# inksci/TRPO

Measured on AMD Instinct MI355X. Metric: TRPO updates/sec (10-iter CG + linesearch) at N states; FVP GB/s vs HBM peak, higher is better.
Workload: dtype fp32 (f16x3 split); 1 GPU; C4: 8M states, obs 128, 256x256 tanh MLP, 18 actions; full update = discount+standardise+pg+10 CG+shs FVP+line search+final losses; n_states=8000000, obs_dim=128, n_actions=18, num_params=103442, cg_iters=10, parallelism=dp1 (row shards, RCCL all-reduce of [P] FVP/grad + loss scalars)

## Files before the change

include/trpo_engine.h:

```cpp
#ifndef TRPO_ENGINE_H
#define TRPO_ENGINE_H

#include <stdint.h>

#ifdef __cplusplus
extern "C" {
#endif

#define TRPO_MEM_HOST 0
#define TRPO_MEM_DEVICE 1

#define TRPO_OK 0
#define TRPO_ERR_ARG (-1)
#define TRPO_ERR_HIP (-2)
#define TRPO_ERR_RCCL (-3)
#define TRPO_ERR_STATE (-4)

typedef struct trpo_engine trpo_engine;

typedef struct trpo_update_params {
  int cg_iters;
  float residual_tol;
  float cg_damping;
  double max_kl;
// ... 9 lines not shown
  double shs, lm, rate;
  float surr_before, kl_before, ent_before;
  float surr_after, kl_after, ent_after;
  float rdotr;
  float gdotstepdir;
} trpo_update_stats;

#define TRPO_VEC_THETA 0
#define TRPO_VEC_THETA_PREV 1
#define TRPO_VEC_G 2
#define TRPO_VEC_STEPDIR 3
#define TRPO_VEC_FULLSTEP 4
#define TRPO_VEC_THETA_LS 5


int trpo_create(trpo_engine** out, int obs_dim, const int* hidden, int n_hidden, int n_actions,
                int64_t max_rows, int device);
void trpo_destroy(trpo_engine* e);
const char* trpo_last_error(void);
int64_t trpo_num_params(const trpo_engine* e);
int trpo_synchronize(trpo_engine* e);
void* trpo_stream(trpo_engine* e);

int trpo_comm_unique_id(uint8_t out_id[128]);
int trpo_comm_init(trpo_engine* e, const uint8_t id[128], int rank, int world);
typedef int (*trpo_allreduce_cb)(void* host_buf, int64_t count, int dtype, void* ctx);
int trpo_comm_set_host_allreduce(trpo_engine* e, trpo_allreduce_cb cb, void* ctx, int rank, int world);
typedef struct trpo_comm_info_t {
  int transport;
  int rank, world;
  int comm_count, comm_rank, comm_device;
  int device;
  char pci_bus_id[64];
} trpo_comm_info_t;
int trpo_comm_info(trpo_engine* e, trpo_comm_info_t* out);

int trpo_set_flat(trpo_engine* e, const float* theta, int mem);
int trpo_get_flat(trpo_engine* e, float* theta_out, int mem);
int trpo_get_vector(trpo_engine* e, int which, float* out, int mem);

int trpo_set_batch(trpo_engine* e, int64_t n, int64_t n_global, const float* states,
                   const int64_t* actions, const float* advant, const float* old_dist, int mem);
int trpo_set_rewards(trpo_engine* e, const double* rewards, const uint8_t* episode_starts,
                     const double* baseline, int mem);
int trpo_compute_advantages(trpo_engine* e, double gamma, double* returns_out, double* advant_out,
                            int mem);

int trpo_standardize(trpo_engine* e, double* adv, int64_t n, int64_t n_global, float* adv32_out, int mem);

#define TRPO_ADV_RETURNS 0
#define TRPO_ADV_GAE 1
int trpo_set_advantage_estimator(trpo_engine* e, int kind, double lambda);
int trpo_get_advantage_estimator(trpo_engine* e, int* kind, double* lambda);
int trpo_set_tail_values(trpo_engine* e, const double* tail_values, int mem);
int trpo_get_tail_values(trpo_engine* e, double* out, int mem);

int trpo_losses(trpo_engine* e, float out3[3]);
int trpo_eval_losses(trpo_engine* e, const float* theta, float out3[3], int mem);
int trpo_action_dist(trpo_engine* e, float* out, int mem);
int trpo_policy_grad(trpo_engine* e, float* g_out, int mem);
int trpo_fvp(trpo_engine* e, const float* v, float* out, float damping, int mem);

int trpo_cg(trpo_engine* e, const float* b, float* x_out, int cg_iters, float residual_tol,
            float damping, int* iters_out, int mem);
#define TRPO_F32 0
#define TRPO_F64 1
typedef int (*trpo_fax_cb)(const void* p, void* z, void* ctx);
int trpo_cg_callback(trpo_fax_cb f_Ax, void* ctx, const void* b, void* x_out, int64_t n, int dtype,
                     int cg_iters, double residual_tol, int* iters_out);
int trpo_linesearch(trpo_engine* e, const float* x, const float* fullstep, double expected_improve_rate,
                    float* theta_out, int* k_out, int mem);

void trpo_default_params(trpo_update_params* p);
int trpo_update(trpo_engine* e, const trpo_update_params* p, trpo_update_stats* stats);

int trpo_device_count(int* out);
int trpo_discount(const double* x, const uint8_t* episode_starts, int64_t n, double gamma,
                  double* out, int mem);
int trpo_gae(const double* rewards, const double* values, const uint8_t* episode_starts,
             const double* tail_values, int64_t n, double gamma, double lambda, double* adv_out,
             double* returns_out, int mem);

int trpo_set_option(const char* name, int value);
int trpo_get_option(const char* name, int* value);

int trpo_profile_enable(trpo_engine* e, int enable);
int trpo_profile_query(trpo_engine* e, char* buf, int cap);
int trpo_profile_reset(trpo_engine* e);

typedef struct trpo_rollout_params {
  int n_envs;
  int max_pathlength;
  int64_t n_timesteps;
  int train;
  int time_limit;
  uint64_t seed;
  const double* reset_uniforms;
  const double* action_uniforms;
  int max_episodes_per_env;
  int mem;
} trpo_rollout_params;
void trpo_default_rollout_params(trpo_rollout_params* p);
int trpo_rollout_cartpole(trpo_engine* e, const trpo_rollout_params* p, int64_t* n_steps_out, int64_t* n_paths_out);
int trpo_rollout_fetch(trpo_engine* e, double* obs, float* obs32, int64_t* actions, float* action_dists,
                       double* rewards, uint8_t* episode_starts, double* uniforms, int mem);
int trpo_rollout_fetch_ends(trpo_engine* e, uint8_t* truncated, double* final_obs, float* final_dists,
                            int64_t* lengths, int64_t* end_rows, int mem);
int trpo_rollout_to_batch(trpo_engine* e, int64_t n_global);
typedef struct trpo_feed_view {
  int64_t n, n_global;
  int obs_dim, n_actions;
  const float* states;
  int ld_states;
  const float* old_dist;
  int ld_old;
  const uint8_t* episode_starts;
  const double* returns;
  double* baseline;
} trpo_feed_view;
int trpo_get_feed_view(trpo_engine* e, trpo_feed_view* out);
typedef struct trpo_tail_view {
  int64_t n, n_paths;
  int obs_dim, n_actions;
  const float* final_obs32;
  const float* final_dist;
  const int64_t* lengths;
  const uint8_t* truncated;
  const int64_t* end_rows;
  double* tail;
} trpo_tail_view;
int trpo_get_tail_view(trpo_engine* e, trpo_tail_view* out);
int trpo_set_baseline(trpo_engine* e, const double* baseline, int mem);
int trpo_explained_variance(trpo_engine* e, double* out);
int trpo_act(trpo_engine* e, const float* states, int64_t n, const double* uniforms, int train, int64_t* actions_out,
             float* dists_out, int mem);
int trpo_cat_sample(const float* prob, int64_t n, int k, const double* uniforms, int64_t* out, int mem);
int trpo_cartpole_step(const double* state, const int64_t* action, int64_t n, double* state_out, double* reward,
                       uint8_t* done, int mem);

typedef struct trpo_vf trpo_vf;
int trpo_vf_create(trpo_vf** out, int feat_dim, const int* hidden, int n_hidden, int64_t max_rows, int device);
void trpo_vf_destroy(trpo_vf* vf);
int64_t trpo_vf_num_params(const trpo_vf* vf);
int trpo_vf_set_params(trpo_vf* vf, const float* flat, int mem);
int trpo_vf_get_params(trpo_vf* vf, float* flat_out, int mem);
int trpo_vf_set_adam(trpo_vf* vf, float lr, float beta1, float beta2, float epsilon);
int trpo_vf_reset_optimizer(trpo_vf* vf);
int trpo_vf_get_optimizer(trpo_vf* vf, float* m_out, float* v_out, float powers_out[2], int64_t* steps_out,
                          int mem);
int trpo_vf_set_features(trpo_vf* vf, int64_t n, int64_t n_global, const float* obs, int obs_dim,
                         const float* action_dists, int n_actions, const uint8_t* episode_starts, int mem);
int trpo_vf_set_features_view(trpo_vf* vf, const trpo_feed_view* view, int with_targets);
int trpo_vf_set_feature_matrix(trpo_vf* vf, int64_t n, int64_t n_global, const float* feat, int mem);
int trpo_vf_get_feature_matrix(trpo_vf* vf, float* feat_out, int mem);
int trpo_vf_set_targets(trpo_vf* vf, const void* returns, int dtype, int mem);
int trpo_vf_fit(trpo_vf* vf, int steps);
int trpo_vf_gradient(trpo_vf* vf, float* grad_out, double* loss_out, int mem);
int trpo_vf_predict(trpo_vf* vf, void* out, int dtype, int mem);
int trpo_vf_predict_tails(trpo_vf* vf, const trpo_tail_view* view);
int trpo_vf_comm_init(trpo_vf* vf, const uint8_t id[128], int rank, int world);
int trpo_vf_comm_set_host_allreduce(trpo_vf* vf, trpo_allreduce_cb cb, void* ctx, int rank, int world);

#ifdef __cplusplus
}
#endif
#endif
// ... 1 lines not shown
```

trpo_amd/_lib.py:

```python
from __future__ import annotations

import ctypes
import os
from ctypes import (CFUNCTYPE, POINTER, byref, c_char_p, c_double, c_float, c_int, c_int64, c_uint8,
                    c_void_p)

HERE = os.path.dirname(os.path.abspath(__file__))
LIB_PATH = os.environ.get("TRPO_ENGINE_LIB", os.path.join(HERE, "libtrpo_engine.so"))

MEM_HOST = 0
MEM_DEVICE = 1

VEC_THETA, VEC_THETA_PREV, VEC_G, VEC_STEPDIR, VEC_FULLSTEP, VEC_THETA_LS = range(6)

ADV_RETURNS, ADV_GAE = 0, 1


class UpdateParams(ctypes.Structure):
    _fields_ = [("cg_iters", c_int), ("residual_tol", c_float), ("cg_damping", c_float),
                ("max_kl", c_double), ("compute_advantages", c_int), ("gamma", c_double)]


class UpdateStats(ctypes.Structure):
    _fields_ = [("cg_iters", c_int), ("k", c_int), ("reverted", c_int), ("pad", c_int),
                ("shs", c_double), ("lm", c_double), ("rate", c_double),
                ("surr_before", c_float), ("kl_before", c_float), ("ent_before", c_float),
                ("surr_after", c_float), ("kl_after", c_float), ("ent_after", c_float),
                ("rdotr", c_float), ("gdotstepdir", c_float)]

    def as_dict(self):
        return {name: getattr(self, name) for name, _ in self._fields_ if name != "pad"}


class RolloutParams(ctypes.Structure):
    _fields_ = [("n_envs", c_int), ("max_pathlength", c_int), ("n_timesteps", c_int64), ("train", c_int),
                ("time_limit", c_int), ("seed", ctypes.c_uint64), ("reset_uniforms", c_void_p),
                ("action_uniforms", c_void_p), ("max_episodes_per_env", c_int), ("mem", c_int)]


class CommInfo(ctypes.Structure):
    _fields_ = [("transport", c_int), ("rank", c_int), ("world", c_int), ("comm_count", c_int),
                ("comm_rank", c_int), ("comm_device", c_int), ("device", c_int), ("pci_bus_id", ctypes.c_char * 64)]


class FeedView(ctypes.Structure):
    _fields_ = [("n", c_int64), ("n_global", c_int64), ("obs_dim", c_int), ("n_actions", c_int),
                ("states", c_void_p), ("ld_states", c_int), ("old_dist", c_void_p), ("ld_old", c_int),
                ("episode_starts", c_void_p), ("returns", c_void_p), ("baseline", c_void_p)]


class TailView(ctypes.Structure):
    _fields_ = [("n", c_int64), ("n_paths", c_int64), ("obs_dim", c_int), ("n_actions", c_int),
                ("final_obs32", c_void_p), ("final_dist", c_void_p), ("lengths", c_void_p),
                ("truncated", c_void_p), ("end_rows", c_void_p), ("tail", c_void_p)]


FAX_CB = CFUNCTYPE(c_int, c_void_p, c_void_p, c_void_p)
ALLREDUCE_CB = CFUNCTYPE(c_int, c_void_p, c_int64, c_int, c_void_p)
F32, F64 = 0, 1

SIGNATURES = {
    "trpo_create": (c_int, [POINTER(c_void_p), c_int, POINTER(c_int), c_int, c_int, c_int64, c_int]),
    "trpo_destroy": (None, [c_void_p]),
    "trpo_last_error": (c_char_p, []),
    "trpo_num_params": (c_int64, [c_void_p]),
    "trpo_synchronize": (c_int, [c_void_p]),
    "trpo_stream": (c_void_p, [c_void_p]),
    "trpo_comm_unique_id": (c_int, [POINTER(c_uint8)]),
    "trpo_comm_init": (c_int, [c_void_p, POINTER(c_uint8), c_int, c_int]),
    "trpo_comm_set_host_allreduce": (c_int, [c_void_p, ALLREDUCE_CB, c_void_p, c_int, c_int]),
    "trpo_comm_info": (c_int, [c_void_p, ctypes.POINTER(CommInfo)]),
    "trpo_set_flat": (c_int, [c_void_p, c_void_p, c_int]),
    "trpo_get_flat": (c_int, [c_void_p, c_void_p, c_int]),
    "trpo_get_vector": (c_int, [c_void_p, c_int, c_void_p, c_int]),
    "trpo_set_batch": (c_int, [c_void_p, c_int64, c_int64, c_void_p, c_void_p, c_void_p, c_void_p, c_int]),
    "trpo_set_rewards": (c_int, [c_void_p, c_void_p, c_void_p, c_void_p, c_int]),
    "trpo_compute_advantages": (c_int, [c_void_p, c_double, c_void_p, c_void_p, c_int]),
    "trpo_standardize": (c_int, [c_void_p, c_void_p, c_int64, c_int64, c_void_p, c_int]),
    "trpo_set_advantage_estimator": (c_int, [c_void_p, c_int, c_double]),
    "trpo_get_advantage_estimator": (c_int, [c_void_p, POINTER(c_int), POINTER(c_double)]),
    "trpo_set_tail_values": (c_int, [c_void_p, c_void_p, c_int]),
    "trpo_get_tail_values": (c_int, [c_void_p, c_void_p, c_int]),
    "trpo_losses": (c_int, [c_void_p, POINTER(c_float)]),
    "trpo_eval_losses": (c_int, [c_void_p, c_void_p, POINTER(c_float), c_int]),
    "trpo_action_dist": (c_int, [c_void_p, c_void_p, c_int]),
    "trpo_policy_grad": (c_int, [c_void_p, c_void_p, c_int]),
    "trpo_fvp": (c_int, [c_void_p, c_void_p, c_void_p, c_float, c_int]),
    "trpo_cg": (c_int, [c_void_p, c_void_p, c_void_p, c_int, c_float, c_float, POINTER(c_int), c_int]),
    "trpo_cg_callback": (c_int, [FAX_CB, c_void_p, c_void_p, c_void_p, c_int64, c_int, c_int, c_double,
                                 POINTER(c_int)]),
    "trpo_linesearch": (c_int, [c_void_p, c_void_p, c_void_p, c_double, c_void_p, POINTER(c_int), c_int]),
    "trpo_default_params": (None, [POINTER(UpdateParams)]),
    "trpo_update": (c_int, [c_void_p, POINTER(UpdateParams), POINTER(UpdateStats)]),
    "trpo_device_count": (c_int, [POINTER(c_int)]),
    "trpo_discount": (c_int, [c_void_p, c_void_p, c_int64, c_double, c_void_p, c_int]),
    "trpo_gae": (c_int, [c_void_p, c_void_p, c_void_p, c_void_p, c_int64, c_double, c_double, c_void_p, c_void_p,
                         c_int]),
    "trpo_set_option": (c_int, [c_char_p, c_int]),
    "trpo_get_option": (c_int, [c_char_p, POINTER(c_int)]),
    "trpo_profile_enable": (c_int, [c_void_p, c_int]),
    "trpo_profile_query": (c_int, [c_void_p, c_char_p, c_int]),
    "trpo_profile_reset": (c_int, [c_void_p]),
    "trpo_default_rollout_params": (None, [POINTER(RolloutParams)]),
    "trpo_rollout_cartpole": (c_int, [c_void_p, POINTER(RolloutParams), POINTER(c_int64), POINTER(c_int64)]),
    "trpo_rollout_fetch": (c_int, [c_void_p, c_void_p, c_void_p, c_void_p, c_void_p, c_void_p, c_void_p, c_void_p,
                                   c_int]),
    "trpo_rollout_fetch_ends": (c_int, [c_void_p, c_void_p, c_void_p, c_void_p, c_void_p, c_void_p, c_int]),
    "trpo_get_tail_view": (c_int, [c_void_p, POINTER(TailView)]),
    "trpo_vf_predict_tails": (c_int, [c_void_p, POINTER(TailView)]),
    "trpo_set_baseline": (c_int, [c_void_p, c_void_p, c_int]),
    "trpo_get_feed_view": (c_int, [c_void_p, POINTER(FeedView)]),
    "trpo_vf_set_features_view": (c_int, [c_void_p, POINTER(FeedView), c_int]),
    "trpo_explained_variance": (c_int, [c_void_p, POINTER(c_double)]),
    "trpo_rollout_to_batch": (c_int, [c_void_p, c_int64]),
    "trpo_act": (c_int, [c_void_p, c_void_p, c_int64, c_void_p, c_int, c_void_p, c_void_p, c_int]),
    "trpo_cat_sample": (c_int, [c_void_p, c_int64, c_int, c_void_p, c_void_p, c_int]),
    "trpo_cartpole_step": (c_int, [c_void_p, c_void_p, c_int64, c_void_p, c_void_p, c_void_p, c_int]),
    "trpo_vf_create": (c_int, [POINTER(c_void_p), c_int, POINTER(c_int), c_int, c_int64, c_int]),
    "trpo_vf_destroy": (None, [c_void_p]),
    "trpo_vf_num_params": (c_int64, [c_void_p]),
    "trpo_vf_set_params": (c_int, [c_void_p, c_void_p, c_int]),
    "trpo_vf_get_params": (c_int, [c_void_p, c_void_p, c_int]),
    "trpo_vf_set_adam": (c_int, [c_void_p, c_float, c_float, c_float, c_float]),
    "trpo_vf_reset_optimizer": (c_int, [c_void_p]),
    "trpo_vf_get_optimizer": (c_int, [c_void_p, c_void_p, c_void_p, POINTER(c_float), POINTER(c_int64), c_int]),
    "trpo_vf_set_features": (c_int, [c_void_p, c_int64, c_int64, c_void_p, c_int, c_void_p, c_int, c_void_p,
                                     c_int]),
    "trpo_vf_set_feature_matrix": (c_int, [c_void_p, c_int64, c_int64, c_void_p, c_int]),
    "trpo_vf_get_feature_matrix": (c_int, [c_void_p, c_void_p, c_int]),
    "trpo_vf_set_targets": (c_int, [c_void_p, c_void_p, c_int, c_int]),
    "trpo_vf_fit": (c_int, [c_void_p, c_int]),
    "trpo_vf_gradient": (c_int, [c_void_p, c_void_p, POINTER(c_double), c_int]),
    "trpo_vf_predict": (c_int, [c_void_p, c_void_p, c_int, c_int]),
    "trpo_vf_comm_init": (c_int, [c_void_p, POINTER(c_uint8), c_int, c_int]),
    "trpo_vf_comm_set_host_allreduce": (c_int, [c_void_p, ALLREDUCE_CB, c_void_p, c_int, c_int]),
}


class EngineError(RuntimeError):
    pass


def _load():
    if not os.path.isfile(LIB_PATH):
        raise ImportError(
            f"trpo_amd: HIP engine library not found at {LIB_PATH}; build it with "
            f"`python -c 'import __graft_entry__ as g; g.build()'` (there is no CPU fallback)")
    try:
        lib = ctypes.CDLL(LIB_PATH)
    except OSError as exc:
        raise ImportError(f"trpo_amd: failed to load {LIB_PATH}: {exc}") from exc
    for name, (res, args) in SIGNATURES.items():
        fn = getattr(lib, name)
        fn.restype = res
        fn.argtypes = args
    return lib


lib = _load()


def check(rc: int, what: str = ""):
    if rc != 0:
        msg = lib.trpo_last_error()
        raise EngineError(f"{what} failed (rc={rc}): {msg.decode() if msg else ''}")
    return rc


def device_count() -> int:
    n = c_int(0)
    check(lib.trpo_device_count(ctypes.byref(n)), "trpo_device_count")
    return n.value


def set_option(name: str, value: int):
    check(lib.trpo_set_option(name.encode(), int(value)), f"trpo_set_option({name})")


def get_option(name: str) -> int:
    out = c_int(0)
    check(lib.trpo_get_option(name.encode(), byref(out)), f"trpo_get_option({name})")
# ... 2 lines not shown
```

trpo_amd/csrc/engine.cpp:

```cpp
#include "../../include/trpo_engine.h"
#include "abi_util.h"
#include "common.h"
#include "kernels.h"

#include <hip/hip_runtime.h>
#include <rccl/rccl.h>

#include <algorithm>
#include <cmath>
#include <cstddef>
#include <cstdio>
#include <cstdlib>
#include <cstring>
#include <map>
#include <memory>
#include <stdexcept>
#include <string>
#include <type_traits>
#include <vector>

using namespace trpo;

using namespace trpo_abi;

// ... 81 lines not shown
    void rd_written() { ds_ready = false; }
  } cache;

  bool f16 = false;
  unsigned* amax = nullptr;
  unsigned* am(int group, int l) const {
    return f16 ? amax + (size_t)(1 + group * kMaxLayers + l) * kAmaxSlot : nullptr;
  }
  unsigned* am_x() const { return f16 ? amax : nullptr; }
  unsigned* am_w(int l) const { return am(0, l); }
  unsigned* am_v(int l) const { return am(1, l); }
  unsigned* am_d(int l) const { return am(3, l); }
  unsigned* am_ds(int l) const { return am(4, l); }
  unsigned* am_rh(int l) const { return am(5, l); }
  unsigned* am_rd(int l) const { return am(6, l); }
  void am_reset(unsigned* first, int count) {
    if (first && count > 0)
      HIPCHECK(hipMemsetAsync(first, 0, (size_t)count * kAmaxSlot * sizeof(unsigned), stream));
  }
  uint16_t *Xh = nullptr, *Xl = nullptr, *W0b = nullptr, *V0b = nullptr;
  int* pl_e = nullptr;
  uint16_t* D1h = nullptr;
  int d1_ldp = 0;
  int* eD1t = nullptr;
  bool use_hbwd2() const {
    return g_options.hbwd2 != 0 && L >= 3 && wp[L - 1] > 128 && head_bwd2_eligible(w[L], wp[L - 1]);
  }
  int x_mpad = 0, x_ldp = 0;
  bool x_planes = false;
  bool planes_geom_l0() const {
    return L >= 2 && wp[1] % 256 == 0 && r16(wp[0]) % 64 == 0;
  }
  bool f16_split() const { return f16 && split_on(); }
  bool x_planes_on() const { return x_planes && g_options.planes != 0 && split_on(); }
  bool planes_l0() const { return x_planes_on() && planes_geom_l0() && rowgemm_uses_split(wp[1], RowEpi::kTanh); }
  bool rbwd0_geom() const { return L >= 2 && rbwd0_eligible(wp[0], (wp[0] + 63) / 64 * 64, wp[1], wp[2]); }
  void attach_x_planes(GemmSeg& sg, uint16_t* dst) {
    launch_block_planes(sg.B3, 2, wp[1], r16(wp[0]), dst, stream);
    sg.Ah = Xh;
    sg.Al = Xl;
    sg.ldp = x_ldp;
    sg.mpad = x_mpad;
    sg.eAp = pl_e;
    sg.Bb = dst;
  }
  uint16_t* tail_planes = nullptr;
  bool use_tail() const {
    return g_options.tail != 0 && f16_split() && L >= 2 && tail_eligible(wp[L - 1], wp[L]) && w[L] <= 32;
  }
  bool e_top_needed() const { return L < 2 || !use_tail() || use_fused() || use_chain(); }
  void reprepare_if_path_changed() {
    if (cache.prepared && ((e_top_needed() && !cache.prep_e_top) || cache.prep_fused16 != use_fused16()))
      cache.prepared = false;
  }

  struct ImageSet {
    uint16_t* img = nullptr;
    int* tab = nullptr;
    int* e = nullptr;
    int nchunks = 0;
    ChainImgArgs jobs{};
  };
  int chain_otm = 0;
  ImageSet chain_set;
  bool use_fused() const { return g_options.fused != 0 && chain_otm > 0 && fused_fvp_eligible(L, w.data()); }
  ImageSet f16_set;
  bool f16_v_img_ready = false;
  unsigned* cg_ticket = nullptr;
  ImageSet f16_loss_set;
  bool use_fused16() const { return g_options.fused == 3 && f16 && f16_set.img && fused16_eligible(L, w.data()); }
  uint16_t* rf_img = nullptr;
  uint16_t* fw_img = nullptr;
  bool use_rfwd01() const {
    return g_options.rfwd01 != 0 && rf_img && f16_split() && use_tail() && planes_l0() &&
           rfwd01_eligible(L, w.data(), wp.data()) && rfwd01_rows_ok(x_mpad);
  }
  bool use_fwd01() const {
    return g_options.fwd01 != 0 && fw_img && f16_split() && planes_l0() && fwd01_eligible(L, w.data(), wp.data()) &&
           rfwd01_rows_ok(x_mpad);
  }
  bool use_rbwd0() const {
    return g_options.rbwd0 != 0 && f16 && x_planes_on() && rbwd0_geom() && rowgemm_uses_split(wp[1], RowEpi::kRBwd);
  }
  RBwd0Args rbwd0_args(const int* skip) const {
    RBwd0Args a{};
    a.rows = (int)n;
    a.K = wp[2];
    a.lda = wp[2];
    a.N = w[1];
    a.Npad = wp[1];
    a.obs = w[0];
    a.B0 = WB3[1];
    a.B1 = WB3[1] + 3 * plane3_b(1);
    a.ldk = r16(wp[2]);
    a.plane = (int64_t)plane3_b(1);
    a.am_b0 = am_w(1);
    a.am_b1 = am_v(1);
    a.H = H[1];
    a.Xh = Xh;
    a.Xl = Xl;
    a.x_mpad = x_mpad;
    a.x_ldp = x_ldp;
    a.eX = pl_e;
    a.dst = slab_dst(0);
    a.skip = skip;
    return a;
  }
  bool use_chain() const {
    return chain_otm > 0 && (g_options.chain >= 2 || (g_options.chain == 1 && chain_otm <= 8));
  }

  struct RollBufs {
    std::vector<void*> mem;
    int64_t rows = 0;
    int envs = 0;
    double* obs = nullptr;
    int64_t* actions = nullptr;
    float* dist = nullptr;
    double* rewards = nullptr;
    uint8_t* starts = nullptr;
    double* uniforms = nullptr;
    int64_t *counts = nullptr, *episodes = nullptr, *offsets = nullptr;
    double *reset_u = nullptr, *act_u = nullptr;
    int64_t reset_u_n = 0, act_u_n = 0;
    int64_t paths = 0;
    uint8_t* end_truncated = nullptr;
    double* end_obs = nullptr;
    float* end_dist = nullptr;
    int64_t *end_len = nullptr, *end_row = nullptr, *path_offsets = nullptr;
    uint8_t* cat_truncated = nullptr;
    float *cat_obs32 = nullptr, *cat_dist = nullptr;
    int64_t *cat_len = nullptr, *cat_rows = nullptr;
  } roll;
  RolloutArgs roll_args{};
  int64_t roll_n = 0, roll_paths = 0, roll_maxcount = 0, roll_maxpaths = 0;
  bool roll_valid = false;
  bool feed_is_rollout = false;

  bool prof = false;
  struct Ev {
    std::string tag;
    hipEvent_t a, b;
  };
  std::vector<Ev> ev_live;
  std::vector<hipEvent_t> ev_pool;
  std::map<std::string, std::pair<long, double>> prof_acc;

  template <class T>
  T* dalloc(size_t count) {
    void* ptr = nullptr;
    const size_t bytes = std::max<size_t>(count * sizeof(T), 16);
    HIPCHECK(hipMalloc(&ptr, bytes));
    HIPCHECK(hipMemsetAsync(ptr, 0, bytes, stream));
    allocs.push_back(ptr);
    return static_cast<T*>(ptr);
  }

  void use() {
    HIPCHECK(hipSetDevice(device));
    if (!har_slots.empty()) rewind_har();
  }

  const float* act_in(int l) const { return l == 0 ? X : H[l]; }

  hipEvent_t take_event() {
    if (!ev_pool.empty()) {
// ... 18 lines not shown
      if (e->prof) begin(std::string(prefix) + "_l" + std::to_string(l));
    }
    void begin(const std::string& tag) {
      Ev ev{tag, e->take_event(), e->take_event()};
      HIPCHECK(hipEventRecord(ev.a, e->stream));
      e->ev_live.push_back(ev);
      idx = (int)e->ev_live.size() - 1;
    }
    ~Scope() {
      if (idx >= 0) (void)hipEventRecord(e->ev_live[idx].b, e->stream);
    }
  };
  void prof_collect() {
    if (ev_live.empty()) return;
    HIPCHECK(hipStreamSynchronize(stream));
    for (auto& ev : ev_live) {
      float ms = 0.f;
      HIPCHECK(hipEventElapsedTime(&ms, ev.a, ev.b));
      auto& acc = prof_acc[ev.tag];
      acc.first += 1;
      acc.second += ms;
      ev_pool.push_back(ev.a);
      ev_pool.push_back(ev.b);
    }
    ev_live.clear();
  }

  void init(int obs, const int* hidden, int nh, int A, int64_t max_rows, int dev) {
    REQUIRE(obs > 0 && A > 0 && nh >= 0 && max_rows > 0, "invalid policy dimensions");
    REQUIRE(nh + 1 <= kMaxLayers, "too many layers");
    REQUIRE(A <= 32 * kMaxHeadTiles, "n_actions must be <= 128 (softmax rows of up to 4 x 32 lanes)");
    REQUIRE(max_rows < (int64_t(1) << 31), "max_rows must fit in int32 row indices");
    for (int i = 0; i < nh; ++i) REQUIRE(hidden[i] > 0, "hidden widths must be positive");
    device = dev;
    use();
    HIPCHECK(hipDeviceGetAttribute(&num_cus, hipDeviceAttributeMultiprocessorCount, device));
    HIPCHECK(hipStreamCreateWithFlags(&stream, hipStreamNonBlocking));
    w.push_back(obs);
    for (int i = 0; i < nh; ++i) w.push_back(hidden[i]);
    w.push_back(A);
    L = (int)w.size() - 1;
    for (int v : w) wp.push_back(pad4(v));
    P = 0;
    for (int l = 0; l < L; ++l) {
      offW.push_back(P);
      P += (int64_t)w[l] * w[l + 1];
      offb.push_back(P);
      P += w[l + 1];
    }
    cap = max_rows;

    for (float** v : {&theta, &theta_prev, &theta_trial, &theta_ls, &g, &bneg, &x, &r, &p, &p2, &z, &hv,
                      &stepdir, &fullstep, &vin, &vout})
      *v = dalloc<float>(P);
    int maxpad = 4;
    for (int l = 0; l < L; ++l) {
      WF.push_back(dalloc<float>((size_t)2 * wp[l] * wp[l + 1]));
      WB.push_back(dalloc<float>((size_t)2 * wp[l + 1] * wp[l]));
      WFt.push_back(dalloc<float>((size_t)2 * wp[l] * wp[l + 1]));
      maxpad = std::max<int>(maxpad, 2 * wp[l] * wp[l + 1]);
    }
    WBt_scratch = dalloc<float>(maxpad);
    for (int l = 0; l < L; ++l) {
      WF3.push_back(dalloc<uint16_t>(2 * plane3_f(l) * 3));
      WB3.push_back(dalloc<uint16_t>(2 * plane3_b(l) * 3));
      WFt3.push_back(dalloc<uint16_t>(plane3_f(l) * 3));
    }
    X = dalloc<float>((size_t)cap * wp[0]);
    act = dalloc<int>(cap);
    adv32 = dalloc<float>(cap);
    old = dalloc<float>((size_t)cap * wp[L]);
    rewards = dalloc<double>(cap);
    returns = dalloc<double>(cap);
    adv64 = dalloc<double>(cap);
    baseline = dalloc<double>(cap);
    starts = dalloc<uint8_t>(cap);
    H.assign(L + 1, nullptr);
    RH.assign(L + 1, nullptr);
    D.assign(L, nullptr);
    RD.assign(L, nullptr);
    E.assign(L, nullptr);
    for (int l = 1; l < L; ++l) {
      H[l] = dalloc<float>((size_t)cap * wp[l]);
      RH[l] = dalloc<float>((size_t)cap * wp[l]);
    }
    for (int l = 0; l < L; ++l) {
      D[l] = dalloc<float>((size_t)cap * wp[l + 1]);
      RD[l] = dalloc<float>((size_t)cap * wp[l + 1]);
      if (l < L - 1) E[l] = dalloc<float>((size_t)cap * wp[l + 1]);
    }
    Pm = dalloc<float>((size_t)cap * wp[L]);
    DSL = dalloc<float>((size_t)cap * wp[L]);
    rowterms = dalloc<double>((size_t)cap * 4);
    int tiles_max = 1;
    for (int l = 0; l < L; ++l)
      tiles_max = std::max(tiles_max, ((w[l] + 255) / 256) * ((w[l + 1] + 255) / 256));
    slab_stride = (P + 63) / 64 * 64;
    int s_target = std::max(1, std::min(512, 1024 / tiles_max));
    if (tiles_max == 1)
      s_target = (int)std::max<int64_t>(s_target, std::min<int64_t>(2048, (int64_t(128) << 20) / (slab_stride * 4)));
    const int64_t slab_bytes = (int64_t)slab_stride * 4;
    auto fit = [&](int64_t bytes) { return std::max<int64_t>(1, bytes / slab_bytes); };
    s_target = (int)std::max<int64_t>(s_target, std::min<int64_t>(fit(int64_t(2) << 30), (cap + 16383) / 16384));
    if (tiles_max == 1 && s_target == 512 && num_cus < 512 && (cap + 16383) / 16384 <= num_cus) s_target = num_cus;
    if (g_options.splits > 0) s_target = std::min(g_options.splits, 8192);
    int s_pg = (int)std::max<int64_t>(
        s_target, std::min<int64_t>({2048, std::max<int64_t>(4 * (int64_t)s_target, (cap + 4095) / 4096),
                                     fit(int64_t(8) << 30)}));
    if (g_options.pg_splits > 0) s_pg = std::min(g_options.pg_splits, 8192);
    slab = dalloc<float>((size_t)std::max(s_target, s_pg) * slab_stride);
    S = s_target;
    S_pg = s_pg;
    S_cur = S;
    partA = dalloc<double>(kRedBlocks * 3);
    partB = dalloc<double>(kRedBlocks * 3);
    part3 = dalloc<double>(kRedBlocks * 3);
    local3 = dalloc<double>(4);
    dscal = dalloc<double>(8);
    scan_ws = dalloc<uint8_t>(std::max(discount_workspace_bytes(cap), gae_workspace_bytes(cap)));
    sc = dalloc<UpdScalars>(1);
    fl = dalloc<CGFlags>(1);
    cg_ticket = dalloc<unsigned>(1);
    dbad = dalloc<int>(1);
    f16 = g_options.split_f16 != 0;
    amax = dalloc<unsigned>((size_t)(1 + 8 * kMaxLayers) * kAmaxSlot);
    if (L >= 2 && tail_eligible(wp[L - 1], wp[L])) tail_planes = dalloc<uint16_t>((size_t)2 * 2 * 32 * kTailK);
    if (rfwd01_eligible(L, w.data(), wp.data())) rf_img = dalloc<uint16_t>(rfwd01_img_bytes() / 2);
    if (fwd01_eligible(L, w.data(), wp.data())) fw_img = dalloc<uint16_t>(fwd01_img_bytes() / 2);
    stage = dalloc<float>((size_t)cap * std::max(std::max(wp[0], wp[L]), 2));
    if (f16 && (planes_geom_l0() || rbwd0_geom())) {
      x_ldp = (wp[0] + 63) / 64 * 64;
      const size_t xp = (size_t)((cap + 255) / 256 * 256) * x_ldp;
      Xh = dalloc<uint16_t>(xp);
      Xl = dalloc<uint16_t>(xp);
      W0b = dalloc<uint16_t>(2 * plane3_f(0));
      V0b = dalloc<uint16_t>(2 * plane3_f(0));
      pl_e = dalloc<int>(8);
    }
    if (f16 && L >= 2 && rbwd0_geom()) {
      d1_ldp = (wp[2] + 31) / 32 * 32;
      D1h = dalloc<uint16_t>((size_t)((cap + 255) / 256 * 256) * d1_ldp);
      eD1t = dalloc<int>((size_t)(cap + 31) / 32 + 8);
    }
    HIPCHECK(hipHostMalloc((void**)&hsc, sizeof(UpdScalars), hipHostMallocDefault));
    std::memset(hsc, 0, sizeof(UpdScalars));
    setup_chain();
    setup_fused16();
    HIPCHECK(hipStreamSynchronize(stream));
  }

  struct ImgJob {
    int l, trans, which;
  };
  struct ImgGeom {
    int kc, otp, csz;
  };
  std::vector<ImgJob> fvp_image_order() const {
    std::vector<ImgJob> order = {ImgJob{0, 0, 1}};
    for (int l = 1; l < L; ++l) {
      order.push_back({l, 0, 0});
      order.push_back({l, 0, 1});
    }
    for (int l = L - 1; l >= 1; --l) {
      order.push_back({l, 1, 0});
      order.push_back({l, 1, 1});
    }
    return order;
// ... 555 lines not shown
      if (l == L - 1 && hb2) {
        am_reset(am_ds(L - 2), 1);
        HeadBwd2Args hb{};
        hb.rows = (int)n;
        hb.A = w[L];
        hb.Apad = wp[L];
        hb.N = w[L - 1];
        hb.Npad = wp[L - 1];
        hb.WB = WB[L - 1];
        hb.D2 = D[L - 1];
        hb.DS2 = DSL;
        hb.H = H[L - 1];
        hb.D1 = D[L - 2];
        hb.DS1 = RD[L - 2];
        hb.E1 = prep_e_top ? E[L - 2] : nullptr;
        hb.am_d1 = am_d(L - 2);
        hb.am_ds1 = am_ds(L - 2);
        PgSplits pgs(this);
        hb.dst = slab_dst(L - 1);
        if (L == 3 && D1h && eD1t && use_rbwd0() && wp[2] % 32 == 0 && n > 0) {
          cache.d1_mpad = (int)((n + 255) / 256 * 256);
          hb.D1h = D1h;
          hb.d1_mpad = cache.d1_mpad;
          hb.eD1t = eD1t;
        }
        Scope sp(this, "bwd2_l2");
        launch_head_bwd2(hb, num_cus, stream);
        check_launch();
        cache.ds_ready = true;
        cache.d1_plane = cache.d1_tiled = hb.D1h != nullptr;
        continue;
      }
      RowGemmArgs a = row_args(w[l], wp[l]);
      a.nseg = 1;
      a.seg[0] = bwd_seg(l, kW, D[l], am_d(l));
      a.epi = need_d ? (need_e ? RowEpi::kPrepBwd : RowEpi::kPgBwd) : RowEpi::kPrepBwdE;
      a.ea.H = H[l];
      a.ea.out0 = need_d ? D[l - 1] : E[l - 1];
      a.ea.amax0 = need_d ? am_d(l - 1) : nullptr;
      a.ea.out1 = need_d && need_e ? E[l - 1] : nullptr;
      a.ea.ldo = wp[l];
      Scope sp(this, "bwd", l);
      launch_rowgemm(a, stream);
      check_launch();
    }
    if (!cache.d1_plane && D1h && use_rbwd0() && n > 0) {
      cache.d1_mpad = (int)((n + 255) / 256 * 256);
      Scope sp(this, "split_d1");
      launch_split_planes(D[1], (int)n, cache.d1_mpad, wp[2], wp[2], D1h, nullptr, d1_ldp, am_d(1), pl_e + 1, stream);
      check_launch();
      cache.d1_plane = true;
    }
    reduce_losses(0, nullptr);
    cache.prepared = true;
  }

  void reduce_grad(float* out, const int* skip, int slabs = 0) {
    {
      Scope sp(this, "reduce");
      launch_reduce_slab(slab, slabs > 0 ? slabs : active_splits, slab_stride, P, out, skip, stream);
      check_launch();
    }
    allreduce_f32(out, (size_t)P);
  }

  void wgrad_layer(int l, int nseg, WSeg s0, WSeg s1, int colsum_seg, const int* skip, const char* tag) {
    WGradArgs a{};
    a.rows = (int)n;
    a.Ma = w[l];
    a.Nb = w[l + 1];
    a.Mpad = wp[l];
    a.Npad = wp[l + 1];
    a.nseg = nseg;
    a.seg[0] = s0;
    a.seg[1] = s1;
    a.colsum_seg = colsum_seg;
    a.dst = slab_dst(l);
    a.skip = skip;
    a.f16 = f16;
    Scope sp(this, tag, l);
    launch_wgrad(a, stream);
    check_launch();
  }
  void fvp_wgrads(int l0, int l1, const int* skip) {
    for (int l = l0; l < l1; ++l) {
      if (l == 0)
        wgrad_layer(0, 1, WSeg{X, RD[0], wp[0], wp[1], am_x(), am_rd(0)}, WSeg{}, 0, skip, "fvp_wgrad");
      else
        wgrad_layer(l, 2, WSeg{RH[l], D[l], wp[l], wp[l + 1], am_rh(l), am_d(l)},
                    WSeg{H[l], RD[l], wp[l], wp[l + 1], nullptr, am_rd(l)}, 1, skip, "fvp_wgrad");
    }
  }

  void policy_grad() {
    reprepare_if_path_changed();
    prepare();
    if (use_fused16()) {
      if (!cache.pg_ready) pg_fused16();
      reduce_grad(g, nullptr, cache.pg_grid);
      return;
    }
    ensure_w3();
    PgSplits pgs(this);
    cache.slabs_written(true);
    std::vector<float*> DS(L);
    DS[L - 1] = DSL;
    for (int l = 0; l < L - 1; ++l) DS[l] = RD[l];
    const bool have_ds = cache.ds_ready;
    am_reset(am_ds(0), have_ds ? L - 2 : L - 1);
    const bool r0f = use_rbwd0();
    for (int l = have_ds ? L - 2 : L - 1; l >= 1; --l) {
      if (l == 1 && r0f) {
        RBwd0Args a = rbwd0_args(nullptr);
        a.nseg = 1;
        a.A0 = DS[1];
        a.am_a0 = am_ds(1);
        Scope sp(this, "pg_bwdwg_l1");
        launch_rbwd0(a, stream);
        check_launch();
        continue;
      }
      RowGemmArgs a = row_args(w[l], wp[l]);
      a.nseg = 1;
      a.seg[0] = bwd_seg(l, kW, DS[l], am_ds(l));
      a.epi = RowEpi::kPgBwd;
      a.ea.H = H[l];
      a.ea.out0 = DS[l - 1];
      a.ea.amax0 = am_ds(l - 1);
      a.ea.ldo = wp[l];
      Scope sp(this, "pg_bwd", l);
      launch_rowgemm(a, stream);
      check_launch();
    }
    for (int l = r0f ? 1 : 0; l < (have_ds ? L - 1 : L); ++l)
      wgrad_layer(l, 1, WSeg{act_in(l), DS[l], wp[l], wp[l + 1], l == 0 ? am_x() : nullptr, am_ds(l)}, WSeg{}, 0,
                  nullptr, "pg_wgrad");
    reduce_grad(g, nullptr);
  }

  void fvp(const float* v, float* out, const int* skip, int* defer = nullptr) {
    if (defer) *defer = 0;
    reprepare_if_path_changed();
    prepare();
    cache.rd_written();
    cache.slabs_written();
    if (use_fused16()) {
      fvp_fused16(v, out, skip, defer && !multi_rank() && cg_fused_reduce_ok(P) ? defer : nullptr);
      return;
    }
    if (use_fused()) {
      fvp_fused(v, out, skip);
      return;
    }
    if (use_chain()) {
      fvp_chain(v, out, skip);
      return;
    }
    {
      PackArgs pa = pack_args(WF, &WB, 1);
      launch_pack(pa, v, 1, skip, stream);
      check_launch();
    }
    ensure_w3();
    split_parts(false, true, false, true, cur_set(), skip, "split_v");
    am_reset(am_rh(0), L);
    am_reset(am_rd(0), L);
    const bool tail = use_tail();
    const int Lf = tail ? L - 1 : L;
    int l_first = 0;
    if (use_rfwd01()) {
      {
        Scope sp(this, "fvp_rfwd_img");
        launch_rfwd01_img(theta, v, offW[0], offW[1], w[0], am_v(0), am_w(1), am_v(1), rf_img, skip, stream);
        check_launch();
      }
      Rfwd01Args ra{};
      ra.n = n;
      ra.obs = w[0];
      ra.ldh = wp[1];
      ra.ldz = wp[2];
      ra.Xh = Xh;
      ra.Xl = Xl;
      ra.x_mpad = x_mpad;
      ra.eX = pl_e;
      ra.H1 = H[1];
      ra.c0 = v + offb[0];
      ra.c1 = v + offb[1];
      ra.V0 = v + offW[0];
      ra.RH1 = RH[1];
      ra.RZ2 = RH[2];
      ra.img = rf_img;
      ra.am_v0 = am_v(0);
      ra.am_w1 = am_w(1);
      ra.am_v1 = am_v(1);
      ra.am_rh1 = am_rh(1);
      ra.am_rz2 = am_rh(2);
      ra.skip = skip;
      Scope sp(this, "fvp_rfwd01");
      launch_rfwd01(ra, num_cus, stream);
      check_launch();
      l_first = 2;
    }
    for (int l = l_first; l < Lf; ++l) {
      RowGemmArgs a = row_args(w[l + 1], wp[l + 1]);
      if (l == 0) {
        a.nseg = 1;
        a.seg[0] = fwd_seg(0, kV, X, am_x(), cur_set());
        if (planes_l0()) attach_x_planes(a.seg[0], V0b);
      } else {
        a.nseg = 2;
        a.seg[0] = fwd_seg(l, kW, RH[l], am_rh(l), cur_set());
        a.seg[1] = fwd_seg(l, kV, H[l], nullptr, cur_set());
      }
      a.skip = skip;
      a.ea.bias = v + offb[l];
      a.ea.ldo = wp[l + 1];
      if (l < L - 1) {
        a.epi = (tail && l == L - 2) ? RowEpi::kRZ : RowEpi::kRHidden;
        a.ea.H = H[l + 1];
        a.ea.out0 = RH[l + 1];
        a.ea.amax0 = am_rh(l + 1);
      } else {
        a.epi = RowEpi::kRHead;
        a.ea.P = Pm;
        a.ea.out0 = RD[L - 1];
        a.ea.amax0 = am_rd(L - 1);
        a.ea.invN = 1.0 / (double)n_global;
      }
      Scope sp(this, "fvp_rfwd", l);
      launch_rowgemm(a, stream);
      check_launch();
    }
    if (tail) {
      const int l = L - 1;
      TailPackArgs tp{};
      tp.theta = theta;
      tp.v = v;
      tp.off_w = offW[l];
      tp.a = w[l];
      tp.b = w[l + 1];
      tp.am_w = am_w(l);
      tp.am_v = am_v(l);
      tp.out = tail_planes;
      TailArgs ta{};
      ta.rows = (int)n;
      ta.a = w[l];
      ta.b = w[l + 1];
      ta.apad = wp[l];
      ta.bpad = wp[l + 1];
      ta.RH = RH[l];
      ta.rz = 1;
      ta.H = H[l];
      ta.P = Pm;
      ta.DL = D[l];
      ta.c = v + offb[l];
      ta.WV16 = tail_planes;
      ta.WT16 = WB3[l];
      ta.VT16 = WB3[l] + 3 * plane3_b(l);
      ta.bplane = (int64_t)plane3_b(l);
      ta.am_rh = am_rh(l);
      ta.am_d = am_d(l);
      ta.am_w = am_w(l);
      ta.am_v = am_v(l);
      ta.am_out = am_rd(l - 1);
      ta.RDout = RD[l - 1];
      ta.invN = 1.0 / (double)n_global;
      ta.dst = slab_dst(l);
      ta.skip = skip;
      Scope sp(this, "fvp_tail", l);
      launch_tail_pack(tp, stream);
      launch_fvp_tail(ta, stream);
      check_launch();
    }
    const bool r0f = use_rbwd0() && Lf - 1 >= 1;
    for (int l = Lf - 1; l >= 1; --l) {
      if (l == 1 && r0f) {
        RBwd0Args a = rbwd0_args(skip);
        a.nseg = 2;
        a.A0 = RD[1];
        a.A1 = D[1];
        if (cache.d1_plane) {
          a.A1h = D1h;
          a.a1_mpad = cache.d1_mpad;
          a.eA1p = pl_e + 1;
          if (cache.d1_tiled) a.eA1t = eD1t;
        }
        a.am_a0 = am_rd(1);
        a.am_a1 = am_d(1);
        a.E = E[0];
        a.RH = RH[1];
        Scope sp(this, "fvp_rbwdwg_l1");
        launch_rbwd0(a, stream);
        check_launch();
        continue;
      }
      RowGemmArgs a = row_args(w[l], wp[l]);
      a.nseg = 2;
      a.seg[0] = bwd_seg(l, kW, RD[l], am_rd(l));
      a.seg[1] = bwd_seg(l, kV, D[l], am_d(l));
      a.skip = skip;
      a.epi = RowEpi::kRBwd;
      a.ea.H = H[l];
      a.ea.E = E[l - 1];
      a.ea.RH = RH[l];
      a.ea.out0 = RD[l - 1];
      a.ea.amax0 = am_rd(l - 1);
      a.ea.ldo = wp[l];
      Scope sp(this, "fvp_rbwd", l);
      launch_rowgemm(a, stream);
      check_launch();
    }
    fvp_wgrads(r0f ? 1 : 0, Lf, skip);
    reduce_grad(out, skip);
  }

  ChainArgs chain_args(const ImageSet& is, const float* v, const int* skip) const {
    ChainArgs ca{};
    ca.n = (int)n;
    ca.L = L;
    for (int l = 0; l <= L; ++l) {
      ca.w[l] = w[l];
      ca.ld[l] = wp[l];
    }
    ca.X = X;
    for (int l = 0; l < L; ++l) {
      ca.H[l] = H[l];
      ca.RH[l] = RH[l];
      ca.D[l] = D[l];
      ca.E[l] = E[l];
      ca.RD[l] = RD[l];
      ca.offb[l] = offb[l];
    }
    ca.P = Pm;
    ca.v = v;
    ca.img = is.img;
    ca.tab = is.tab;
    ca.nchunks = is.nchunks;
    ca.invN = 1.0 / (double)n_global;
    ca.skip = skip;
    return ca;
  }
  void chain_w_images(const float* v) {
    if (cache.chain_w_valid) return;
    Scope sp(this, "fvp_img_w");
    launch_chain_img(chain_set.jobs, theta, v, 0, nullptr, stream);
    check_launch();
    cache.chain_w_valid = true;
  }
  void chain_images(const float* v, const int* skip) {
    chain_w_images(v);
    Scope sp(this, "fvp_img_v");
    launch_chain_img(chain_set.jobs, theta, v, 1, skip, stream);
    check_launch();
  }

  void fvp_fused(const float* v, float* out, const int* skip) {
    chain_images(v, skip);
    const int variant = g_options.fused == 1 ? 1 : 2;
    const int rb = fused_fvp_states_per_group(variant);
    FusedArgs fa{};
    fa.c = chain_args(chain_set, v, skip);
    fa.slab = slab;
    fa.slab_stride = slab_stride;
    for (int l = 0; l < L; ++l) fa.offW[l] = offW[l];
    fa.ngroups = (int)((n + rb - 1) / rb);
    const int per_cu = variant == 2 ? 2 : 1;
    const int grid =
        (int)std::max<int64_t>(1, std::min<int64_t>({(int64_t)fa.ngroups, (int64_t)S, (int64_t)num_cus * per_cu}));
    {
      Scope sp(this, "fvp_fused");
      launch_fvp_fused(fa, grid, variant, stream);
      check_launch();
    }
    reduce_grad(out, skip, grid);
  }

  Fused16Args fused16_args(const float* v, const int* skip, int& grid) {
    const int rb = fused16_states_per_group();
    Fused16Args fa{};
    fa.f.c = chain_args(f16_set, v, skip);
    fa.f.slab = slab;
    fa.f.slab_stride = slab_stride;
    for (int l = 0; l < L; ++l) fa.f.offW[l] = offW[l];
    fa.f.ngroups = (int)((n + rb - 1) / rb);
    fa.img_e = f16_set.e;
    fa.am_x = am_x();
    fa.am_d1 = am_d(1);
    fa.am_d2 = L == 3 ? am_d(2) : nullptr;
    fa.DS = DSL;
    fa.am_ds2 = am_ds(L - 1);
    const int64_t slots = std::max<int64_t>(
        1, std::min<int64_t>({(int64_t)fa.f.ngroups, (int64_t)S, (int64_t)num_cus * fused16_groups_per_cu()}));
    const int64_t rounds = (fa.f.ngroups + slots - 1) / slots;
    grid = (int)std::max<int64_t>(1, (fa.f.ngroups + rounds - 1) / rounds);
    return fa;
// ... 1083 lines not shown
```

trpo_amd/csrc/gemm.hip:

```cpp
#include "common.h"
#include "kernels.h"
#include <cstdlib>
#include <stdexcept>
#include <type_traits>
#include <string>

#include "rowepi.h"

namespace trpo {

static int env_int(const char* name, int dflt) {
  const char* e = std::getenv(name);
  return e ? std::atoi(e) : dflt;
}
Options g_options = {env_int("TRPO_SPLIT_MFMA", 5), env_int("TRPO_SPLIT_WG", 1), env_int("TRPO_CHAIN", 1),
                     env_int("TRPO_SPLIT_F16", 1), env_int("TRPO_SPLIT_MIN_K", 0), env_int("TRPO_GRAPHS", 1),
                     env_int("TRPO_TAIL", 1), env_int("TRPO_FUSED", 3), env_int("TRPO_LOW_SEG", 14),
                     env_int("TRPO_PLANES", 1), env_int("TRPO_RBWD0", 1), env_int("TRPO_HBWD2", 2),
                     env_int("TRPO_HEAD_FWD", 1), env_int("TRPO_SPLITS", 0),
                     env_int("TRPO_PG_SPLITS", 0), env_int("TRPO_LS_FUSED", 1),
                     env_int("TRPO_CG_FUSE_REDUCE", 1), env_int("TRPO_CG_P_IMG", 1),
                     env_int("TRPO_RFWD01", 1), env_int("TRPO_FWD01", 1)};

namespace {

template <int WM, int WN, int TM, int TN, int BK, int EPI, int PF = 1>
__global__ void __launch_bounds__(WM* WN * 64, (TM * TN >= 8 || EPI == 2) ? 2 : 4)
rowgemm_kernel(const RowGemmArgs args) {
  constexpr int BM = WM * TM * 32, BN = WN * TN * 32, NT = WM * WN * 64;
  constexpr int LDA = BK + 4;
  constexpr int LDB = BN + 4;
  constexpr int ASZ = BM * LDA, BSZ = BK * LDB;
  __shared__ __attribute__((aligned(16))) float smem[2 * (ASZ + BSZ)];
  if (args.skip && *args.skip) return;

  const int tid = threadIdx.x, lane = tid & 63, wave = tid >> 6;
  const int wm = wave % WM, wn = wave / WM;
  const int lr = lane & 31, lh = lane >> 5;
  int mt, ntile;
  tile_of((args.Npad + BN - 1) / BN, mt, ntile);
  const int m0 = mt * BM, n0 = ntile * BN;
  const int M = args.M;

  const int nt0 = (args.seg[0].K + BK - 1) / BK;
  const int nt1 = args.nseg > 1 ? (args.seg[1].K + BK - 1) / BK : 0;
  const int ntiles = nt0 + nt1;

  f32x16 acc[TM][TN];
#pragma unroll
  for (int i = 0; i < TM; ++i)
#pragma unroll
    for (int j = 0; j < TN; ++j) acc[i][j] = f32x16{};

  constexpr int AF4 = BM * BK / 4, BF4 = BK * BN / 4;
  constexpr int AP = (AF4 + NT - 1) / NT, BP = (BF4 + NT - 1) / NT;
  struct Stage {
    f32x4 ra[AP], rb[BP];
    bool oka[AP], okb[BP];
  };

  auto gload = [&](Stage& st, int t) {
    const bool s1 = t >= nt0;
    const float* Ap = s1 ? args.seg[1].A : args.seg[0].A;
    const float* Bp = s1 ? args.seg[1].B : args.seg[0].B;
    const int lda = s1 ? args.seg[1].lda : args.seg[0].lda;
    const int ldb = s1 ? args.seg[1].ldb : args.seg[0].ldb;
    const int K = s1 ? args.seg[1].K : args.seg[0].K;
    const int k0 = (s1 ? t - nt0 : t) * BK;
#pragma unroll
    for (int i = 0; i < AP; ++i) {
      const int f = tid + i * NT;
      const int r = f / (BK / 4), kq = f % (BK / 4);
      const int row = m0 + r, k = k0 + 4 * kq;
      const bool ok = (AF4 % NT == 0 || f < AF4) && row < M && k < K;
      st.ra[i] = *reinterpret_cast<const f32x4*>(Ap + (size_t)(ok ? row : 0) * lda + (ok ? k : 0));
      st.oka[i] = ok;
    }
#pragma unroll
    for (int i = 0; i < BP; ++i) {
      const int f = tid + i * NT;
      const int kr = f / (BN / 4), cq = f % (BN / 4);
      const int k = k0 + kr, col = n0 + 4 * cq;
      const bool ok = (BF4 % NT == 0 || f < BF4) && k < K && col < args.Npad;
      st.rb[i] = *reinterpret_cast<const f32x4*>(Bp + (size_t)(ok ? k : 0) * ldb + (ok ? col : 0));
      st.okb[i] = ok;
    }
  };
  auto sstore = [&](const Stage& st, int buf) {
    float* As = smem + buf * (ASZ + BSZ);
    float* Bs = As + ASZ;
#pragma unroll
    for (int i = 0; i < AP; ++i) {
      const int f = tid + i * NT;
      if (AF4 % NT == 0 || f < AF4) {
        const int r = f / (BK / 4), kq = f % (BK / 4);
        *reinterpret_cast<f32x4*>(As + r * LDA + 4 * kq) = st.oka[i] ? st.ra[i] : f32x4{};
      }
    }
#pragma unroll
    for (int i = 0; i < BP; ++i) {
      const int f = tid + i * NT;
      if (BF4 % NT == 0 || f < BF4) {
        const int kr = f / (BN / 4), cq = f % (BN / 4);
        *reinterpret_cast<f32x4*>(Bs + kr * LDB + 4 * cq) = st.okb[i] ? st.rb[i] : f32x4{};
      }
// ... 240 lines not shown
          c = __builtin_amdgcn_mfma_f32_32x32x16_bf16(a[1], b[1], c, 0, 0, 0);
          c = __builtin_amdgcn_mfma_f32_32x32x16_bf16(a[2], b[0], c, 0, 0, 0);
          c = __builtin_amdgcn_mfma_f32_32x32x16_bf16(a[0], b[2], c, 0, 0, 0);
          c = __builtin_amdgcn_mfma_f32_32x32x16_bf16(a[1], b[0], c, 0, 0, 0);
          c = __builtin_amdgcn_mfma_f32_32x32x16_bf16(a[0], b[1], c, 0, 0, 0);
          c = __builtin_amdgcn_mfma_f32_32x32x16_bf16(a[0], b[0], c, 0, 0, 0);
          acc[tm][tn] = c;
        }
      } else {
        f16x8 b[2];
#pragma unroll
        for (int p = 0; p < 2; ++p) b[p] = *reinterpret_cast<const f16x8*>(Bs + p * BPL + bo);
#pragma unroll
        for (int tm = 0; tm < TM; ++tm) {
          f16x8 a[2];
          const int ao = swk(wm * TM * 32 + tm * 32 + lr, 2 * ks + lh);
#pragma unroll
          for (int p = 0; p < 2; ++p) a[p] = *reinterpret_cast<const f16x8*>(As + p * APL + ao);
          f32x16 c = acc[tm][tn];
          c = __builtin_amdgcn_mfma_f32_32x32x16_f16(a[1], b[0], c, 0, 0, 0);
          c = __builtin_amdgcn_mfma_f32_32x32x16_f16(a[0], b[1], c, 0, 0, 0);
          c = __builtin_amdgcn_mfma_f32_32x32x16_f16(a[0], b[0], c, 0, 0, 0);
          acc[tm][tn] = c;
        }
      }
    }
  };
  auto compute = [&](int buf, int t) {
    if (t >= nt0 ? one1 : one0) compute_p(buf, std::true_type{});
    else compute_p(buf, std::false_type{});
  };
  auto seg_switch = [&](int t) {
    if constexpr (NP == 2) {
      if (t == nt0 && nt1 > 0) {
        asm volatile("; segment switch" ::: "memory");
        scale_acc<TM, TN>(acc, eP1 - eP0);
      }
    }
  };

  if (ntiles > 0) {
    if constexpr (PF == 1) {
      Stage S;
      gload(S, 0);
      sstore(S, 0);
      lds_barrier();
      for (int t = 0; t < ntiles; ++t) {
        if (t + 1 < ntiles) gload(S, t + 1);
        seg_switch(t);
        compute(t & 1, t);
        if (t + 1 < ntiles) sstore(S, (t + 1) & 1);
        lds_barrier();
      }
    } else {
      Stage S0, S1;
      gload(S0, 0);
      gload(S1, ntiles > 1 ? 1 : 0);
      sstore(S0, 0);
      lds_barrier();
      int t = 0;
      for (; t + 1 < ntiles; t += 2) {
        gload(S0, t + 2 < ntiles ? t + 2 : ntiles - 1);
        seg_switch(t);
        compute(0, t);
        sstore(S1, 1);
        lds_barrier();
        gload(S1, t + 3 < ntiles ? t + 3 : ntiles - 1);
        seg_switch(t + 1);
        compute(1, t + 1);
        if (t + 2 < ntiles) sstore(S0, 0);
        lds_barrier();
      }
      if (t < ntiles) {
        seg_switch(t);
        compute(0, t);
      }
    }
  }
  if constexpr (NP == 2) scale_acc<TM, TN>(acc, -(nt1 > 0 ? eP1 : eP0));
  row_epilogue<WM, WN, TM, TN, EPI>(args, acc, m0, n0, wm, wn, lr, lh);
}


template <int WM, int WN, int TM, int TN, int OCC, int PF, int NP>
__global__ void __launch_bounds__(WM* WN * 64, OCC)
wgrad3_kernel(const WGradArgs args) {
  constexpr int BK = 16;
  constexpr int BM = WM * TM * 32, BN = WN * TN * 32, NT = WM * WN * 64;
  constexpr int APL = BM * BK, BPL = BN * BK;
  constexpr int STG = NP * (APL + BPL);
  __shared__ __attribute__((aligned(16))) unsigned short smem[2 * STG];
  __shared__ float cs_sh[2][BN];
  if (args.skip && *args.skip) return;

  const int tid = threadIdx.x, lane = tid & 63, wave = tid >> 6;
  const int wm = wave % WM, wn = wave / WM;
  const int lr = lane & 31, lh = lane >> 5;
  const int m0 = blockIdx.x * BM, n0 = blockIdx.y * BN, split = blockIdx.z;
  const int r0 = split * args.dst.rows_per_split;
  const int r1 = min(args.rows, r0 + args.dst.rows_per_split);
  const int nk = r1 > r0 ? (r1 - r0 + BK - 1) / BK : 0;
  const int ntiles = nk * args.nseg;
  const bool do_colsum = (blockIdx.x == 0);
  int eA[2] = {0, 0}, eB[2] = {0, 0};
  if constexpr (NP == 2) {
    for (int g = 0; g < args.nseg && g < 2; ++g) {
      eA[g] = amax_exp(args.seg[g].amaxA);
      eB[g] = amax_exp(args.seg[g].amaxB);
    }
  }
  bool one0 = false, one1 = false;
  if constexpr (NP == 2) {
    if (args.low_seg > 0 && args.nseg > 1) {
      const int d = (eA[1] + eB[1]) - (eA[0] + eB[0]);
      const int pen0 = (!args.seg[0].amaxA || !args.seg[0].amaxB) ? 4 : 0;
      const int pen1 = (!args.seg[1].amaxA || !args.seg[1].amaxB) ? 4 : 0;
      one0 = -d >= args.low_seg + pen1;
      one1 = d >= args.low_seg + pen0;
    }
  }

  f32x16 acc[TM][TN];
#pragma unroll
  for (int i = 0; i < TM; ++i)
#pragma unroll
    for (int j = 0; j < TN; ++j) acc[i][j] = f32x16{};

  constexpr int AI = 2 * BM, BI = 2 * BN;
  constexpr int AP = (AI + NT - 1) / NT, BP = (BI + NT - 1) / NT;
  float csum[BP];
#pragma unroll
  for (int i = 0; i < BP; ++i) csum[i] = 0.0f;
  auto desc = [&](const float* p, int ld) {
    return __builtin_amdgcn_make_buffer_rsrc((void*)(p + (size_t)r0 * ld), 0, (r1 - r0) * ld * 4, 0x00020000);
  };
  const int lda4 = args.seg[0].lda * 4, ldb4 = args.seg[0].ldb * 4;
  constexpr int kOob = 0x40000000;
  int vA[AP], vB[BP];
#pragma unroll
  for (int i = 0; i < AP; ++i) {
    const int f = tid + i * NT;
    const int c = f % BM, g = f / BM;
    const bool okc = (AI % NT == 0 || f < AI) && m0 + c < args.Mpad;
    vA[i] = okc ? 8 * g * lda4 + (m0 + c) * 4 : kOob;
  }
#pragma unroll
  for (int i = 0; i < BP; ++i) {
    const int f = tid + i * NT;
    const int c = f % BN, g = f / BN;
    const bool okc = (BI % NT == 0 || f < BI) && n0 + c < args.Npad;
    vB[i] = okc ? 8 * g * ldb4 + (n0 + c) * 4 : kOob;
  }
  auto ldbuf = [](__amdgpu_buffer_rsrc_t r, int vo, int so) {
    return __builtin_bit_cast(float, __builtin_amdgcn_raw_buffer_load_b32(r, vo, so, 0));
  };
  struct Stage {
    float va[AP][8], vb[BP][8];
    bool cs;
    int sg;
  };
  auto gload = [&](Stage& st, int t) {
    const int sg = t / nk;
    const int kt = t - sg * nk;
    st.cs = do_colsum && sg == args.colsum_seg;
    st.sg = sg;
    const __amdgpu_buffer_rsrc_t ra = desc(sg ? args.seg[1].A : args.seg[0].A, args.seg[0].lda);
    const __amdgpu_buffer_rsrc_t rb = desc(sg ? args.seg[1].B : args.seg[0].B, args.seg[0].ldb);
    const int sa = kt * BK * lda4, sb = kt * BK * ldb4;
    __builtin_amdgcn_sched_barrier(0);
#pragma unroll
    for (int i = 0; i < AP; ++i)
#pragma unroll
      for (int q = 0; q < 8; ++q) st.va[i][q] = ldbuf(ra, vA[i], sa + q * lda4);
#pragma unroll
    for (int i = 0; i < BP; ++i)
#pragma unroll
      for (int q = 0; q < 8; ++q) st.vb[i][q] = ldbuf(rb, vB[i], sb + q * ldb4);
    __builtin_amdgcn_sched_barrier(0);
  };
  auto put = [&](unsigned short* base, int plane_elems, int c, int g, const float (&v)[8], int e) {
    unsigned short* dst = base + swz16(c, g);
    if constexpr (NP == 2) {
      const float sc = __builtin_ldexpf(1.0f, e);
      u16x8 h, l;
#pragma unroll
      for (int q = 0; q < 8; ++q) {
        unsigned short hh, ll;
        split2h(v[q] * sc, hh, ll);
        h[q] = hh;
        l[q] = ll;
      }
      *reinterpret_cast<u16x8*>(dst) = h;
      *reinterpret_cast<u16x8*>(dst + plane_elems) = l;
    } else {
      u16x8 h, m, l;
#pragma unroll
      for (int q = 0; q < 8; ++q) {
        unsigned short hh, mm, ll;
        split3(v[q], hh, mm, ll);
        h[q] = hh;
        m[q] = mm;
        l[q] = ll;
      }
      *reinterpret_cast<u16x8*>(dst) = h;
      *reinterpret_cast<u16x8*>(dst + plane_elems) = m;
      *reinterpret_cast<u16x8*>(dst + 2 * plane_elems) = l;
    }
  };
  auto sstore = [&](const Stage& st, int buf) {
    unsigned short* As = smem + buf * STG;
    unsigned short* Bs = As + NP * APL;
#pragma unroll
    for (int i = 0; i < AP; ++i) {
      const int f = tid + i * NT;
      if (AI % NT == 0 || f < AI) put(As, APL, f % BM, f / BM, st.va[i], eA[st.sg]);
    }
#pragma unroll
    for (int i = 0; i < BP; ++i) {
      const int f = tid + i * NT;
      if (BI % NT == 0 || f < BI) {
        put(Bs, BPL, f % BN, f / BN, st.vb[i], eB[st.sg]);
        if (st.cs) {
          float cs = 0.0f;
#pragma unroll
          for (int q = 0; q < 8; ++q) cs += st.vb[i][q];
          csum[i] += cs;
        }
      }
    }
  };
  auto compute_p = [&](int buf, auto one_c) {
    constexpr bool ONE = decltype(one_c)::value;
    const unsigned short* As = smem + buf * STG;
    const unsigned short* Bs = As + NP * APL;
#pragma unroll
    for (int tn = 0; tn < TN; ++tn) {
      const int bo = swz16(wn * TN * 32 + tn * 32 + lr, lh);
      if constexpr (NP == 2 && ONE) {
        const f16x8 b0 = *reinterpret_cast<const f16x8*>(Bs + bo);
#pragma unroll
        for (int tm = 0; tm < TM; ++tm) {
          const int ao = swz16(wm * TM * 32 + tm * 32 + lr, lh);
          const f16x8 a0 = *reinterpret_cast<const f16x8*>(As + ao);
          acc[tm][tn] = __builtin_amdgcn_mfma_f32_32x32x16_f16(a0, b0, acc[tm][tn], 0, 0, 0);
        }
      } else if constexpr (NP == 3) {
        bf16x8 b[3];
#pragma unroll
        for (int p = 0; p < 3; ++p) b[p] = *reinterpret_cast<const bf16x8*>(Bs + p * BPL + bo);
#pragma unroll
        for (int tm = 0; tm < TM; ++tm) {
          bf16x8 a[3];
          const int ao = swz16(wm * TM * 32 + tm * 32 + lr, lh);
#pragma unroll
          for (int p = 0; p < 3; ++p) a[p] = *reinterpret_cast<const bf16x8*>(As + p * APL + ao);
          f32x16 c = acc[tm][tn];
          c = __builtin_amdgcn_mfma_f32_32x32x16_bf16(a[1], b[1], c, 0, 0, 0);
          c = __builtin_amdgcn_mfma_f32_32x32x16_bf16(a[2], b[0], c, 0, 0, 0);
          c = __builtin_amdgcn_mfma_f32_32x32x16_bf16(a[0], b[2], c, 0, 0, 0);
          c = __builtin_amdgcn_mfma_f32_32x32x16_bf16(a[1], b[0], c, 0, 0, 0);
          c = __builtin_amdgcn_mfma_f32_32x32x16_bf16(a[0], b[1], c, 0, 0, 0);
          c = __builtin_amdgcn_mfma_f32_32x32x16_bf16(a[0], b[0], c, 0, 0, 0);
          acc[tm][tn] = c;
        }
      } else {
        f16x8 b[2];
#pragma unroll
        for (int p = 0; p < 2; ++p) b[p] = *reinterpret_cast<const f16x8*>(Bs + p * BPL + bo);
#pragma unroll
        for (int tm = 0; tm < TM; ++tm) {
          f16x8 a[2];
          const int ao = swz16(wm * TM * 32 + tm * 32 + lr, lh);
#pragma unroll
          for (int p = 0; p < 2; ++p) a[p] = *reinterpret_cast<const f16x8*>(As + p * APL + ao);
          f32x16 c = acc[tm][tn];
          c = __builtin_amdgcn_mfma_f32_32x32x16_f16(a[1], b[0], c, 0, 0, 0);
          c = __builtin_amdgcn_mfma_f32_32x32x16_f16(a[0], b[1], c, 0, 0, 0);
          c = __builtin_amdgcn_mfma_f32_32x32x16_f16(a[0], b[0], c, 0, 0, 0);
          acc[tm][tn] = c;
        }
      }
    }
  };
  auto compute = [&](int buf, int t) {
    if (t >= nk ? one1 : one0) compute_p(buf, std::true_type{});
    else compute_p(buf, std::false_type{});
  };
  auto seg_switch = [&](int t) {
    if constexpr (NP == 2) {
      if (t == nk && args.nseg > 1) {
        asm volatile("; segment switch" ::: "memory");
        scale_acc<TM, TN>(acc, (eA[1] + eB[1]) - (eA[0] + eB[0]));
      }
    }
  };

  if (ntiles > 0) {
    if constexpr (PF == 1) {
// ... 265 lines not shown
    }
  if (do_colsum && tid < BN && n0 + tid < args.Nb) out[args.dst.off_b + n0 + tid] = csum;
}

template <int WM, int WN, int TM, int TN, int BKT, int EPI, int PF = 1>
void launch_row_cfg(const RowGemmArgs& a, hipStream_t s) {
  constexpr int BM = WM * TM * 32, BN = WN * TN * 32;
  const long nblk = (long)((a.M + BM - 1) / BM) * ((a.Npad + BN - 1) / BN);
  hipLaunchKernelGGL((rowgemm_kernel<WM, WN, TM, TN, BKT, EPI, PF>), dim3((unsigned)nblk), dim3(WM * WN * 64),
                     0, s, a);
}

template <int WM, int WN, int TM, int TN, int EPI, int OCC = 2, int PF = 1, int BKT = 16>
void launch_row3_cfg(const RowGemmArgs& a, hipStream_t s) {
  constexpr int BM = WM * TM * 32, BN = WN * TN * 32;
  for (int i = 0; i < a.nseg; ++i)
    if (!a.seg[i].B3 || a.seg[i].ldk < ((a.seg[i].K + 15) / 16) * 16 || a.seg[i].ldk % 8)
      throw std::runtime_error("split-bf16 row GEMM: segment without B planes");
  if (a.nseg > 1 && (a.seg[1].lda != a.seg[0].lda || a.seg[1].ldk != a.seg[0].ldk || a.seg[1].plane != a.seg[0].plane))
    throw std::runtime_error("split-bf16 row GEMM: segments with different strides");
  if ((int64_t)BM * a.seg[0].lda * 4 >= (int64_t(1) << 30) || (int64_t)(a.f16 ? 2 : 3) * a.seg[0].plane * 2 >= (int64_t(1) << 30))
    throw std::runtime_error("split-bf16 row GEMM: operand beyond the buffer-descriptor range");
  const long nblk = (long)((a.M + BM - 1) / BM) * ((a.Npad + BN - 1) / BN);
  RowGemmArgs b = a;
  b.low_seg = g_options.low_seg;
  if constexpr (BKT == 32) {
    for (int i = 0; i < a.nseg; ++i)
      if (a.seg[i].ldk % 32) throw std::runtime_error("split row GEMM (BK 32): B planes' ldk not a multiple of 32");
  }
  if (a.f16)
    hipLaunchKernelGGL((rowgemm3_kernel<WM, WN, TM, TN, EPI, OCC, PF, 2, BKT>), dim3((unsigned)nblk),
                       dim3(WM * WN * 64), 0, s, b);
  else if constexpr (BKT == 16)
    hipLaunchKernelGGL((rowgemm3_kernel<WM, WN, TM, TN, EPI, OCC, PF, 3, BKT>), dim3((unsigned)nblk),
                       dim3(WM * WN * 64), 0, s, a);
  else
    throw std::runtime_error("split row GEMM (BK 32): f16 planes only");
}

bool small_k_row(const RowGemmArgs& a) {
  if (g_options.split_min_k <= 0) return false;
  for (int i = 0; i < a.nseg; ++i)
    if (a.seg[i].K >= g_options.split_min_k) return false;
  return true;
}

template <int EPI>
void launch_row_epi(const RowGemmArgs& a, hipStream_t s) {
  if constexpr (epi_is_head(EPI)) {
    if (a.N > 32 * kMaxHeadTiles) throw std::runtime_error("softmax head supports at most 128 actions");
    if (a.N > 64) launch_row_cfg<4, 1, 2, 4, 16, EPI>(a, s);
    else if (a.N > 32) launch_row_cfg<4, 1, 2, 2, 16, EPI>(a, s);
    else launch_row_cfg<4, 1, 2, 1, 16, EPI>(a, s);
  } else if (rowgemm_uses_split(a.Npad, a.epi) && !small_k_row(a)) {
    bool bk32 = a.f16 != 0 && g_options.split_mfma == 5;
    for (int i = 0; i < a.nseg; ++i) bk32 = bk32 && a.seg[i].ldk % 32 == 0;
    if (bk32) launch_row3_cfg<4, 2, 2, 4, EPI, 2, 1, 32>(a, s);
    else if (g_options.split_mfma == 5 || g_options.split_mfma == 6) launch_row3_cfg<4, 2, 2, 4, EPI, 2, 2>(a, s);
    else launch_row3_cfg<2, 4, 2, 2, EPI>(a, s);
  } else {
    if (a.Npad <= 32) launch_row_cfg<4, 1, 2, 1, 16, EPI>(a, s);
    else if (a.Npad <= 64) launch_row_cfg<4, 1, 2, 2, 16, EPI>(a, s);
    else if (a.Npad <= 128) launch_row_cfg<2, 2, 2, 2, 16, EPI>(a, s);
    else launch_row_cfg<2, 4, 2, 2, 16, EPI>(a, s);
  }
}

template <int WM, int WN, int TM, int TN, int BKT = 16, int PF = 1>
void launch_wg_cfg(const WGradArgs& a, hipStream_t s) {
  constexpr int BM = WM * TM * 32, BN = WN * TN * 32;
  dim3 grid((a.Ma + BM - 1) / BM, (a.Nb + BN - 1) / BN, a.dst.splits);
  hipLaunchKernelGGL((wgrad_kernel<WM, WN, TM, TN, BKT, PF>), grid, dim3(WM * WN * 64), 0, s, a);
}

template <int WM, int WN, int TM, int TN, int OCC, int PF>
void launch_wg3_cfg(const WGradArgs& a, hipStream_t s) {
  constexpr int BM = WM * TM * 32, BN = WN * TN * 32;
  if (a.dst.rows_per_split % 16) throw std::runtime_error("split-bf16 wgrad: rows_per_split % 16");
  if (a.nseg > 1 && (a.seg[1].lda != a.seg[0].lda || a.seg[1].ldb != a.seg[0].ldb))
    throw std::runtime_error("split-bf16 wgrad: segments with different leading dimensions");
  if ((int64_t)a.dst.rows_per_split * (a.seg[0].lda > a.seg[0].ldb ? a.seg[0].lda : a.seg[0].ldb) * 4 >= (int64_t(1) << 30))
    throw std::runtime_error("split-bf16 wgrad: a split's rows exceed the 1 GiB buffer-descriptor range");
  dim3 grid((a.Ma + BM - 1) / BM, (a.Nb + BN - 1) / BN, a.dst.splits);
  WGradArgs b = a;
  b.low_seg = g_options.low_seg;
  if (a.f16)
    hipLaunchKernelGGL((wgrad3_kernel<WM, WN, TM, TN, OCC, PF, 2>), grid, dim3(WM * WN * 64), 0, s, b);
  else
    hipLaunchKernelGGL((wgrad3_kernel<WM, WN, TM, TN, OCC, PF, 3>), grid, dim3(WM * WN * 64), 0, s, a);
}

}

bool rowgemm_uses_split(int Npad, RowEpi epi) {
  return g_options.split_mfma != 0 && Npad > 128 && !epi_is_head((int)epi);
}

void launch_split_b(const SplitArgs& a, const int* skip, hipStream_t s) {
  if (a.n <= 0) return;
  int maxb = 1;
  for (int i = 0; i < a.n; ++i) {
    const SplitJob& j = a.job[i];
    if (j.ldk % 8 || j.ldk < ((j.K + 15) / 16) * 16) throw std::runtime_error("split_b: bad ldk");
    const int b = (j.Npad * (j.ldk / 8) + 255) / 256;
    maxb = b > maxb ? b : maxb;
  }
  hipLaunchKernelGGL(split_b_kernel, dim3(maxb, a.n), dim3(256), 0, s, a, skip);
}

void launch_rowgemm(const RowGemmArgs& a, hipStream_t s) {
  if (a.M <= 0) return;
  if (a.seg[0].Ah && g_options.planes != 0 && a.f16 && rowgemm_uses_split(a.Npad, a.epi) && !small_k_row(a) &&
      a.Npad % 256 == 0) {
    launch_rowgemm_planes(a, s);
    return;
  }
  switch (a.epi) {
    case RowEpi::kTanh: launch_row_epi<(int)RowEpi::kTanh>(a, s); break;
    case RowEpi::kRHidden: launch_row_epi<(int)RowEpi::kRHidden>(a, s); break;
    case RowEpi::kRZ: launch_row_epi<(int)RowEpi::kRZ>(a, s); break;
    case RowEpi::kPrepBwd: launch_row_epi<(int)RowEpi::kPrepBwd>(a, s); break;
    case RowEpi::kPgBwd: launch_row_epi<(int)RowEpi::kPgBwd>(a, s); break;
    case RowEpi::kPrepBwdE: launch_row_epi<(int)RowEpi::kPrepBwdE>(a, s); break;
    case RowEpi::kRBwd: launch_row_epi<(int)RowEpi::kRBwd>(a, s); break;
    case RowEpi::kPrepHead: launch_row_epi<(int)RowEpi::kPrepHead>(a, s); break;
    case RowEpi::kLossHead: launch_row_epi<(int)RowEpi::kLossHead>(a, s); break;
    case RowEpi::kRHead: launch_row_epi<(int)RowEpi::kRHead>(a, s); break;
    case RowEpi::kRelu: launch_row_epi<(int)RowEpi::kRelu>(a, s); break;
    case RowEpi::kReluBwd: launch_row_epi<(int)RowEpi::kReluBwd>(a, s); break;
  }
}

void launch_wgrad(const WGradArgs& a, hipStream_t s) {
  if (a.dst.splits <= 0) return;
  const int Mp = a.Ma, Np = a.Nb;
  if (Np <= 32) {
    if (Mp <= 64) launch_wg_cfg<2, 1, 1, 1>(a, s);
    else if (Mp <= 128) launch_wg_cfg<4, 1, 1, 1>(a, s);
    else launch_wg_cfg<4, 1, 2, 1>(a, s);
  } else if (Np <= 64) {
    if (Mp <= 64) launch_wg_cfg<2, 2, 1, 1>(a, s);
    else if (Mp <= 128) launch_wg_cfg<2, 1, 2, 2>(a, s);
    else launch_wg_cfg<4, 1, 2, 2>(a, s);
  } else if (Np <= 128) {
    if (Mp <= 64) launch_wg_cfg<1, 2, 2, 2>(a, s);
    else launch_wg_cfg<2, 2, 2, 2>(a, s);
  } else if (g_options.split_wg != 0) {
    if (Mp <= 128) launch_wg3_cfg<2, 4, 2, 2, 2, 1>(a, s);
    else launch_wg3_cfg<4, 2, 2, 4, 2, 1>(a, s);
  } else {
    if (Mp <= 128) launch_wg_cfg<2, 4, 2, 2>(a, s);
    else launch_wg_cfg<2, 4, 4, 2>(a, s);
  }
}

}
```

trpo_amd/csrc/kernels.h:

```cpp
#pragma once
#include <hip/hip_runtime.h>
#include <cstdint>

namespace trpo {

struct Options {
  int split_mfma;
  int split_wg;
  int chain;
  int split_f16;
  int split_min_k;
  int graphs;
  int tail;
  int fused;
  int low_seg;
  int planes;
  int rbwd0;
  int hbwd2;
  int head_fwd;
  int splits;
  int pg_splits;
  int ls_fused;
  int cg_fuse_reduce;
  int cg_p_img;
  int rfwd01;
  int fwd01;
};

constexpr int kAmaxSub = 256, kAmaxStride = 32, kAmaxSlot = kAmaxSub * kAmaxStride;

__host__ __device__ inline int f16_scale_exp(float m) {
  if (!(m > 0.0f) || !(m < 3.0e38f)) return 0;
  int q = 0;
  (void)frexpf(m, &q);
  int e = 12 - q;
  return e < -100 ? -100 : (e > 100 ? 100 : e);
}
extern Options g_options;

struct GemmSeg {
  const float* A;
  const float* B;
  int lda, ldb, K;
  const uint16_t* B3 = nullptr;
  int ldk = 0, plane = 0;
  const unsigned* amaxA = nullptr;
  const unsigned* amaxB = nullptr;
  const uint16_t* Ah = nullptr;
  const uint16_t* Al = nullptr;
  int ldp = 0, mpad = 0;
  const int* eAp = nullptr;
  const uint16_t* Bb = nullptr;
};

enum class RowEpi : int {
  kTanh = 0,
  kRHidden = 1,
  kPrepBwd = 2,
  kPgBwd = 3,
  kRBwd = 4,
  kPrepHead = 5,
  kLossHead = 6,
  kRHead = 7,
  kRelu = 8,
  kReluBwd = 9,
  kPrepBwdE = 10,
  kRZ = 11,
};
constexpr int kMaxHeadTiles = 4;
constexpr bool epi_is_head(int e) { return e >= (int)RowEpi::kPrepHead && e <= (int)RowEpi::kRHead; }

struct RowEpiArgs {
  const float* bias;
  const float* H;
  const float* E;
  const float* RH;
  float* out0;
  float* out1;
  float* out2;
  int ldo;
  const float* P;
  const float* old;
  const int* act;
  const float* adv;
  double* rowterms;
  double invN;
  unsigned* amax0 = nullptr;
  unsigned* amax1 = nullptr;
  unsigned* amax2 = nullptr;
};

struct RowGemmArgs {
  int M, N, Npad;
  int nseg;
  GemmSeg seg[2];
  const int* skip;
  RowEpi epi;
  RowEpiArgs ea;
  int f16 = 0;
  int low_seg = 0;
};

void launch_rowgemm(const RowGemmArgs& a, hipStream_t s);
void launch_rowgemm_planes(const RowGemmArgs& a, hipStream_t s);
void launch_split_planes(const float* A, int M, int Mpad, int K, int lda, uint16_t* hi, uint16_t* lo, int ldp,
                         const unsigned* amax, int* e_out, hipStream_t s);
void launch_block_planes(const uint16_t* src, int P, int R, int ld, uint16_t* dst, hipStream_t s);
bool rowgemm_uses_split(int Npad, RowEpi epi);

struct SplitJob {
  const float* B;
  uint16_t* B3;
  int K, Npad, ldb, ldk;
  const unsigned* amax = nullptr;
};
constexpr int kMaxSplitJobs = 16;
struct SplitArgs {
  int n;
  SplitJob job[kMaxSplitJobs];
  int f16 = 0;
};
void launch_split_b(const SplitArgs& a, const int* skip, hipStream_t s);

struct SlabDst {
  int splits = 0, rows_per_split = 0;
  float* slab = nullptr;
  int64_t slab_stride = 0;
  int64_t off_w = 0, off_b = 0;
};

struct WSeg {
  const float* A;
  const float* B;
  int lda, ldb;
  const unsigned* amaxA = nullptr;
  const unsigned* amaxB = nullptr;
};

struct WGradArgs {
  int rows;
  int Ma, Nb;
  int Mpad, Npad;
  int nseg;
  WSeg seg[2];
  int colsum_seg;
  SlabDst dst;
  const int* skip;
  int f16 = 0;
  int low_seg = 0;
};

void launch_wgrad(const WGradArgs& a, hipStream_t s);

struct LayerPack {
  int64_t off_w;
  int a, b, apad, bpad;
  float* WF;
  float* WB;
  unsigned* amax = nullptr;
};
constexpr int kMaxLayers = 8;
struct PackArgs {
  int nl;
  LayerPack L[kMaxLayers];
};
void launch_pack(const PackArgs& pa, const float* src, int which, const int* skip, hipStream_t s);

void launch_reduce_slab(const float* slab, int S, int64_t stride, int64_t P, float* out,
                        const int* skip, hipStream_t s);

struct UpdScalars {
  float rdotr[2];
  float alpha, mu;
  int iters;
  int pad0;
  float tol;
  float damping;
  float sdotz;
  float gdots;
  double shs, lm, rate;
  float loss_before[3];
  float loss_trial[3];
  float loss_after[3];
  int accepted, k, reverted, pad1;
  double max_kl;
};
constexpr int kMaxCG = 64;
struct CGFlags {
  int done[kMaxCG + 2];
};

void launch_dot_partials(const float* a, const float* b, int64_t n, double* partials,
                         const int* skip, hipStream_t s);
void launch_cg_init(const float* b, float* x, float* r, float* p, int64_t n, double* partials,
                    UpdScalars* sc, CGFlags* fl, float tol, float damping, hipStream_t s);
void launch_cg_iter(const float* hv, float* x, float* r, float* p, float* z, int64_t n, UpdScalars* sc,
                    double* partials, double* partials2, CGFlags* fl, int it, hipStream_t s);
bool cg_fused_reduce_ok(int64_t P);
void launch_cg_iter_slabs(const float* slab, int S, int64_t stride, float* hv, float* x, float* r, float* p, float* z,
                          int64_t n, UpdScalars* sc, double* partials, double* partials2, CGFlags* fl, int it,
                          hipStream_t s, bool p_update = true);
struct CgStepArgs {
  const float* slab;
  int S, it;
  int64_t stride, P;
  float *hv, *x, *r, *p, *z;
  UpdScalars* sc;
  double* partials;
  CGFlags* fl;
  unsigned* ticket;
};
struct ChainImgArgs;
void launch_cg_step_slabs(const CgStepArgs& a, const ChainImgArgs* img, int* img_e, hipStream_t s);
struct CGScalarsD {
  double rdotr[2];
  double alpha, mu;
  int iters, pad;
  double tol, damping;
};
// ... 116 lines not shown
void launch_fvp_fused16(const Fused16Args& a, int grid, hipStream_t s);
void launch_pg_fused16(const Fused16Args& a, int grid, hipStream_t s);
void launch_prep_pg_fused16(const Fused16Args& a, int grid, hipStream_t s);
struct FwdLoss16Args {
  int64_t n;
  int L = 3;
  int w[4], ld[4];
  const float* X;
  const float* theta;
  int64_t offb[3];
  const void* img;
  const int* tab;
  int nchunks;
  const int* img_e;
  const unsigned* am_x;
  const float* old;
  const int* act;
  const float* adv;
  double* rowterms;
  const int* skip;
  float* H1 = nullptr;
  float* H2 = nullptr;
  float* P = nullptr;
  float* D = nullptr;
  float* DS = nullptr;
  unsigned* am_d = nullptr;
  unsigned* am_ds = nullptr;
  double invN = 0.0;
};
void launch_fwd_loss16(const FwdLoss16Args& a, int num_cus, hipStream_t s);
}

namespace trpo {
constexpr int kTailK = 256;
struct TailArgs {
  int rows, a, b, apad, bpad;
  const float* RH;
  const float* H;
  int rz = 0;
  const float* P;
  const float* DL;
  const float* c;
  const uint16_t* WV16;
  const uint16_t* WT16;
  const uint16_t* VT16;
  int64_t bplane;
  const unsigned *am_rh, *am_d, *am_w, *am_v;
  unsigned* am_out;
  float* RDout;
  double invN;
  SlabDst dst;
  const int* skip;
};
struct TailPackArgs {
  const float* theta;
  const float* v;
  int64_t off_w;
  int a, b;
  const unsigned *am_w, *am_v;
  uint16_t* out;
};
bool tail_eligible(int apad, int bpad);

struct RBwd0Args {
  int rows;
  int K, lda;
  int N, Npad;
  int obs;
  int nseg;
  const float* A0;
  const float* A1;
  const uint16_t* A1h;
  const int* eA1t = nullptr;
  int a1_mpad;
  const int* eA1p;
  const uint16_t* B0;
  const uint16_t* B1;
  int ldk;
  int64_t plane;
  const unsigned *am_a0, *am_b0, *am_a1, *am_b1;
  const float* H;
  const float* E;
  const float* RH;
  const uint16_t* Xh;
  const uint16_t* Xl;
  int x_mpad, x_ldp;
  const int* eX;
  SlabDst dst;
  const int* skip;
  int low_seg = 0;
};
struct HeadBwd2Args {
  int rows;
  int A, Apad;
  int N, Npad;
  const float* WB;
  const float* D2;
  const float* DS2;
  const float* H;
  float* D1;
  float* DS1;
  unsigned* am_d1;
  unsigned* am_ds1;
  uint16_t* D1h = nullptr;
  int d1_mpad = 0;
  int* eD1t = nullptr;
  float* E1 = nullptr;
  SlabDst dst;
};
bool head_bwd2_eligible(int A, int Npad);
struct HeadFwdArgs {
  int64_t rows;
  int A, Apad;
  int K, Kpad;
  const float* H;
  const float* W;
  const float* bias;
  const float* old;
  const int* act;
  const float* adv;
  double* rowterms;
  double invN;
  int prep = 0;
  float* P = nullptr;
  float* D = nullptr;
  float* DS = nullptr;
  unsigned* am_d = nullptr;
  unsigned* am_ds = nullptr;
};
bool head_fwd_eligible(int A, int K);
void launch_head_fwd(const HeadFwdArgs& a, int num_cus, hipStream_t s);
void launch_head_bwd2(const HeadBwd2Args& a, int num_cus, hipStream_t s);
struct Rfwd01Args {
  int64_t n;
  int obs, ldh, ldz;
  const uint16_t *Xh, *Xl;
  int x_mpad;
  const int* eX;
  const float *H1, *c0, *c1;
  const float* V0;
  float *RH1, *RZ2;
  const uint16_t* img;
  const unsigned *am_v0, *am_w1, *am_v1;
  unsigned *am_rh1, *am_rz2;
  const int* skip;
};
struct Fwd01Args {
  int64_t n;
  int obs;
  const uint16_t *Xh, *Xl;
  int x_mpad;
  const int* eX;
  const float *b0, *b1;
  float *H1, *H2;
  const uint16_t* img;
  const unsigned *am_w0, *am_w1;
};
constexpr bool rfwd01_rows_ok(int64_t x_mpad) { return 4 * x_mpad * 64 < (int64_t(1) << 31); }
static_assert(rfwd01_rows_ok((1 << 23) - 256) && !rfwd01_rows_ok(1 << 23), "rfwd01 / fwd01 row limit");
bool fwd01_eligible(int L, const int* w, const int* wp);
size_t fwd01_img_bytes();
void launch_fwd01_img(const float* th, int64_t offW0, int64_t offW1, int obs, const unsigned* am_w0,
                      const unsigned* am_w1, uint16_t* img, hipStream_t s);
void launch_fwd01(const Fwd01Args& a, int num_cus, hipStream_t s);
bool rfwd01_eligible(int L, const int* w, const int* wp);
size_t rfwd01_img_bytes();
void launch_rfwd01_img(const float* theta, const float* v, int64_t offV0, int64_t offW1, int obs,
                       const unsigned* am_v0, const unsigned* am_w1, const unsigned* am_v1, uint16_t* img,
                       const int* skip, hipStream_t s);
void launch_rfwd01(const Rfwd01Args& a, int num_cus, hipStream_t s);
bool rbwd0_eligible(int obs_pad, int x_ldp, int hid_pad, int K);
void launch_rbwd0(const RBwd0Args& a, hipStream_t s);
void launch_tail_pack(const TailPackArgs& p, hipStream_t s);
void launch_fvp_tail(const TailArgs& a, hipStream_t s);
}

namespace trpo {
size_t vf_pos_workspace_bytes(int64_t n);
void launch_vf_features(const float* obs, int obs_dim, int ld_obs, const float* dist, int A, int ld_dist,
                        const uint8_t* starts, int64_t n, int64_t* lastpos, void* ws, float* feat, int Fp,
                        hipStream_t s);
void launch_vf_tail_features(const float* obs, int obs_dim, const float* dist, int A, const int64_t* lengths,
                             int64_t n_paths, float* feat, int Fp, hipStream_t s);
void launch_vf_tail_scatter(const float* pred, const uint8_t* truncated, const int64_t* end_rows, int64_t n_paths,
                            int64_t n, double* tail, hipStream_t s);
struct VFPackArgs {
  int F, H1, H2, H1p, H2p;
  int64_t offW1, offW2;
  float* W1p;
  float* W2p;
  float* W2T;
};
void launch_vf_pack(const VFPackArgs& a, const float* theta, hipStream_t s);
struct VFHeadArgs {
  int64_t n;
  int H2, H2p;
  const float* Z2;
  const float* w3;
  const float* b3;
  int train;
  const float* y;
  float* dout;
  float* dZ2;
  double* loss_rows;
  float* out32;
  double* out64;
};
void launch_vf_head(const VFHeadArgs& a, hipStream_t s);
void launch_adam(float* var, const float* g, float* m, float* v, int64_t n, float alpha, float b1, float b2, float eps,
                 hipStream_t s);
}

namespace trpo {
struct PolicyShape {
  int L;
  int w[kMaxLayers + 1];
  int64_t offW[kMaxLayers], offb[kMaxLayers];
};
struct RolloutArgs {
  PolicyShape ps;
  const float* theta;
  int maxw;
  int n_envs, max_pathlength, time_limit, train;
  int64_t budget;
  int64_t env_cap;
  int max_episodes;
  uint64_t seed;
  const double* reset_u;
  const double* act_u;
  double* obs;
  int64_t* actions;
  float* dist;
  double* rewards;
  uint8_t* starts;
  double* uniforms_out;
  int64_t* counts;
  int64_t* episodes;
  uint8_t* end_truncated;
  double* end_obs;
  float* end_dist;
  int64_t* end_len;
  int64_t* end_row;
// ... 33 lines not shown
```

trpo_amd/csrc/rbwd0.hip:

```cpp
#include "rowepi.h"
#include <stdexcept>
#include <type_traits>

namespace trpo {
namespace {

#ifndef R0_ROWS
#define R0_ROWS 128
#endif
#ifndef R0_EC
#define R0_EC 4
#endif
#ifndef R0_ELA
#define R0_ELA 2
#endif
#ifndef R0_ELA1
#define R0_ELA1 6
#endif
#ifndef R0_NW
#define R0_NW 8
#endif
#ifndef R0_BK
#define R0_BK 32
#endif
#ifndef R0_PF
#if R0_BK == 32
#define R0_PF 2
#else
#define R0_PF 4
#endif
#endif
constexpr int kR0Rows = R0_ROWS;
constexpr int kR0NW = R0_NW;
constexpr int kR0CT = 8 / kR0NW;
constexpr int kR0NT = kR0NW * 64;
constexpr int kR0BK = R0_BK;
constexpr int kR0TM = kR0Rows / 32;
constexpr int kR0XT = 4;
constexpr int kR0APL = kR0Rows * kR0BK;
constexpr int kR0BPL = 256 * kR0BK;
constexpr int kR0STG = 2 * (kR0APL + kR0BPL);
constexpr int kR0XPL = kR0Rows * 128;
constexpr int kR0AI = kR0APL / 4 / kR0NT;
constexpr int kR0BI = 2 * kR0BPL / 8 / kR0NT;
constexpr int kR0XP = 2 * kR0XPL * 2 / 1024;
constexpr int kR0XD = kR0XP / kR0NW;
constexpr bool kR0XAlias = (2 * kR0STG + 2 * kR0XPL) * 2 + 64 > 160 * 1024;
constexpr int kR0LDSU = kR0XAlias ? (2 * kR0STG > 2 * kR0XPL ? 2 * kR0STG : 2 * kR0XPL) : 2 * kR0STG + 2 * kR0XPL;
static_assert(kR0LDSU * 2 <= 160 * 1024, "rbwd0 LDS");
static_assert(kR0BK == 16 || kR0BK == 32, "rbwd0 k-tile");

__device__ __forceinline__ int swzk(int r, int c) {
  if constexpr (kR0BK == 16) return swz16(r, c);
  else return r * 32 + ((c ^ ((r >> 2) & 3)) << 3);
}
static_assert(kR0AI >= 1 && kR0APL % (4 * kR0NT) == 0 && kR0XP % kR0NW == 0, "rbwd0 tile shape");

__device__ __forceinline__ int xoff(int row, int ch) {
  return 2048 * (row >> 3) + 512 * (ch >> 2) + 64 * (row & 7) + 16 * ((ch & 3) ^ ((row >> 2) & 3));
}

__device__ __forceinline__ void dma16(__amdgpu_buffer_rsrc_t rsrc, unsigned voff, unsigned lds) {
  unsigned keep;
  asm volatile("s_mov_b32 %0, m0\n\ts_mov_b32 m0, %3\n\ts_nop 0\n\tbuffer_load_dwordx4 %1, %2, %4 offen lds\n\t"
               "s_mov_b32 m0, %0"
               : "=&s"(keep)
               : "v"(voff), "s"(rsrc), "s"(lds), "s"(0u));
}

#ifndef R0_ABL
#define R0_ABL 0
#endif
typedef short s4 __attribute__((ext_vector_type(4)));
typedef short s8 __attribute__((ext_vector_type(8)));
typedef unsigned u32x4v __attribute__((ext_vector_type(4)));

__device__ __forceinline__ void split8h(const float* x, float s, f16x8& hi, f16x8& lo) {
  typedef __fp16 fp16x2 __attribute__((ext_vector_type(2)));
  u32x4v H, L;
#pragma unroll
  for (int i = 0; i < 4; ++i) {
    const float a = x[2 * i] * s, b = x[2 * i + 1] * s;
    const fp16x2 hp = __builtin_amdgcn_cvt_pkrtz(a, b);
    const fp16x2 lp = __builtin_amdgcn_cvt_pkrtz(a - (float)hp[0], b - (float)hp[1]);
    H[i] = __builtin_bit_cast(unsigned, hp);
    L[i] = __builtin_bit_cast(unsigned, lp);
  }
  hi = __builtin_bit_cast(f16x8, H);
  lo = __builtin_bit_cast(f16x8, L);
}

__device__ __forceinline__ f32x16 mfma3h(const f16x8& ah, const f16x8& al, const f16x8& bh, const f16x8& bl,
                                         f32x16 c) {
  c = __builtin_amdgcn_mfma_f32_32x32x16_f16(al, bh, c, 0, 0, 0);
  c = __builtin_amdgcn_mfma_f32_32x32x16_f16(ah, bl, c, 0, 0, 0);
  return __builtin_amdgcn_mfma_f32_32x32x16_f16(ah, bh, c, 0, 0, 0);
}

template <int NSEG, bool SW>
__device__ __forceinline__ void rbwd0_body(const RBwd0Args& A, unsigned short* smem, float* sMax) {
  constexpr bool kE = NSEG == 2;
  constexpr int TM = kR0TM, CT = kR0CT;

  const int tid0 = threadIdx.x;
  const int r0 = blockIdx.x * A.dst.rows_per_split;
  const int r1 = min(A.rows, r0 + A.dst.rows_per_split);
  const int wv = __builtin_amdgcn_readfirstlane(tid0 >> 6);
  const int Npad = A.Npad, lda = A.lda, K = A.K;
  constexpr int kOob = 0x40000000;

  const int eA0 = amax_exp(A.am_a0), eB0 = amax_exp(A.am_b0);
  const int eA1 = NSEG > 1 ? amax_exp(A.am_a1) : 0, eB1 = NSEG > 1 ? amax_exp(A.am_b1) : 0;
  const int eP = NSEG > 1 ? min(eA0 + eB0, eA1 + eB1) : eA0 + eB0;
  const float sA0 = __builtin_ldexpf(1.0f, eP - eB0), sA1 = __builtin_ldexpf(1.0f, eP - eB1);
  int one1 = 0;
  if (NSEG > 1 && A.low_seg > 0) {
    const int pen0 = (!A.am_a0 || !A.am_b0) ? 4 : 0;
    one1 = __builtin_amdgcn_readfirstlane((eA1 + eB1) - (eA0 + eB0) >= A.low_seg + pen0 ? 1 : 0);
  }
  const int eX = __builtin_amdgcn_readfirstlane(*A.eX);

  const int nk = (K + kR0BK - 1) / kR0BK;
  const int ntiles = NSEG * nk;
  (void)one1;
  constexpr int sw = SW ? 1 : 0;
  const int eA1p = (sw && !A.eA1t) ? __builtin_amdgcn_readfirstlane(*A.eA1p) : 0;
  const int bbytes = (int)(2 * A.plane * 2);

  const unsigned xbytes = (unsigned)A.x_ldp * (unsigned)A.x_mpad * 2u;
  const __amdgpu_buffer_rsrc_t rXh = __builtin_amdgcn_make_buffer_rsrc((void*)A.Xh, 0, xbytes, 0x00020000);
  const __amdgpu_buffer_rsrc_t rXl = __builtin_amdgcn_make_buffer_rsrc((void*)A.Xl, 0, xbytes, 0x00020000);
  unsigned short* const sX = smem + (kR0XAlias ? 0 : 2 * kR0STG);
  const unsigned lds_x = (unsigned)(uintptr_t)sX;

  auto lane_of = [&]() {
    int t = tid0;
    asm volatile("" : "+v"(t));
    return t;
  };
  f32x16 G[kR0XT][CT];
#pragma unroll
  for (int i = 0; i < kR0XT; ++i)
#pragma unroll
    for (int j = 0; j < CT; ++j) G[i][j] = f32x16{};
  int Eacc = 1 << 20;
  float bsum[CT] = {};

  for (int t0 = r0; t0 < r1; t0 += kR0Rows) {
    const int Mt = min(kR0Rows, r1 - t0);
    const int tid = lane_of(), lane = tid & 63, w = tid >> 6;
    const int lr = lane & 31, lh = lane >> 5;
    const int col0 = 32 * CT * w;
    auto xsrc = [&](int kb) {
      const int o = (kb % (kR0XP / 2)) * 1024 + 16 * lane;
      const int row = 8 * (o >> 11) + ((o >> 6) & 7);
      const int ch = 4 * ((o >> 9) & 3) + (((o >> 4) & 3) ^ ((row >> 2) & 3));
      return (unsigned)(((ch >> 2) * A.x_mpad + row) * 32 + 8 * (ch & 3)) * 2u;
    };
    auto x_dma = [&]() {
#pragma unroll
      for (int i = 0; i < kR0XD; ++i) {
        const int kb = kR0XD * wv + i;
        const int pl = kb / (kR0XP / 2);
        dma16(pl ? rXl : rXh, xsrc(kb) + (unsigned)t0 * 64u,
              lds_x + (unsigned)(pl * kR0XPL * 2 + (kb % (kR0XP / 2)) * 1024));
      }
    };
    if (!kR0XAlias) x_dma();

    f32x16 acc[TM][CT];
#pragma unroll
    for (int i = 0; i < TM; ++i)
#pragma unroll
      for (int j = 0; j < CT; ++j) acc[i][j] = f32x16{};
    struct Stage {
      f32x4 ra[kR0AI];
      u16x8 rb[kR0BI];
    };
    auto gload = [&](Stage& st, int t) {
      const bool pt = sw && t < nk;
      const bool s1 = NSEG > 1 && (sw ? t < nk : t >= nk);
      const int kt = (NSEG > 1 && t >= nk) ? t - nk : t;
      const int k0 = kt * kR0BK;
      if (pt) {
        const __amdgpu_buffer_rsrc_t rP = __builtin_amdgcn_make_buffer_rsrc(
            (void*)(A.A1h + ((size_t)kt * A.a1_mpad + t0) * 32), 0, Mt * 64, 0x00020000);
        st.ra[0] = __builtin_bit_cast(f32x4, __builtin_amdgcn_raw_buffer_load_b128(rP, 16 * tid, 0, 0));
      } else {
        const float* Ap = s1 ? A.A1 : A.A0;
        const __amdgpu_buffer_rsrc_t rA =
            __builtin_amdgcn_make_buffer_rsrc((void*)(Ap + (size_t)t0 * lda), 0, Mt * lda * 4, 0x00020000);
#pragma unroll
        for (int i = 0; i < kR0AI; ++i) {
          const int f = tid + i * kR0NT, r = f / (kR0BK / 4), kq = f % (kR0BK / 4);
          const int vo = (k0 + kR0BK > K && k0 + 4 * kq >= K) ? kOob : (r * lda + 4 * kq) * 4;
          st.ra[i] = __builtin_bit_cast(f32x4, __builtin_amdgcn_raw_buffer_load_b128(rA, vo, k0 * 4, 0));
        }
      }
      const __amdgpu_buffer_rsrc_t rB = __builtin_amdgcn_make_buffer_rsrc((void*)(s1 ? A.B1 : A.B0), 0, bbytes,
                                                                          0x00020000);
#pragma unroll
      for (int i = 0; i < kR0BI; ++i) {
        if (pt && i >= kR0BI / 2) break;
        constexpr int CB = kR0BK / 8;
        const int f = tid + i * kR0NT, p = f / (256 * CB), rem = f % (256 * CB), n = rem / CB, kh = rem % CB;
        const int vo = (n < Npad && k0 + 8 * kh < A.ldk) ? (int)((p * A.plane + (int64_t)n * A.ldk + 8 * kh) * 2) : kOob;
        st.rb[i] = __builtin_bit_cast(u16x8, __builtin_amdgcn_raw_buffer_load_b128(rB, vo, k0 * 2, 0));
// ... 65 lines not shown
        for (int j = 0; j < CT; ++j) acc[i][j] = f32x16{} + 1.0f;
    } else {
      const int t1 = sw ? nk : 0;
      int e1s[TM];
#pragma unroll
      for (int i = 0; i < TM; ++i)
        e1s[i] = (sw && A.eA1t) ? __builtin_amdgcn_readfirstlane(A.eA1t[(t0 >> 5) + i]) : eA1p;
#if R0_PF == 4
      Stage S0, S1, S2, S3;
      auto cl = [&](int j) { return j < ntiles ? j : ntiles - 1; };
      gload(S0, 0);
      gload(S1, cl(1));
      gload(S2, cl(2));
      gload(S3, cl(3));
      sstore(S0, 0, 0);
      lds_barrier();
      auto kloop = [&](int tb, int te, auto one_c) {
        for (int t = tb; t < te; t += 4) {
          gload(S0, cl(t + 4));
          compute(0, one_c);
          if (t + 1 < ntiles) sstore(S1, 1, t + 1);
          lds_barrier();
          gload(S1, cl(t + 5));
          if (t + 1 < ntiles) compute(1, one_c);
          if (t + 2 < ntiles) sstore(S2, 0, t + 2);
          lds_barrier();
          gload(S2, cl(t + 6));
          if (t + 2 < ntiles) compute(0, one_c);
          if (t + 3 < ntiles) sstore(S3, 1, t + 3);
          lds_barrier();
          gload(S3, cl(t + 7));
          if (t + 3 < ntiles) compute(1, one_c);
          if (t + 4 < ntiles) sstore(S0, 0, t + 4);
          lds_barrier();
        }
      };
#else
      Stage S0, S1;
      gload(S0, 0);
      gload(S1, ntiles > 1 ? 1 : 0);
      sstore(S0, 0, 0);
      lds_barrier();
      auto kloop = [&](int tb, int te, auto one_c) {
        for (int t = tb; t < te; t += 2) {
          gload(S0, t + 2 < ntiles ? t + 2 : ntiles - 1);
          compute(0, one_c);
          if (t + 1 < ntiles) sstore(S1, 1, t + 1);
          lds_barrier();
          gload(S1, t + 3 < ntiles ? t + 3 : ntiles - 1);
          if (t + 1 < ntiles) compute(1, one_c);
          if (t + 2 < ntiles) sstore(S0, 0, t + 2);
          lds_barrier();
        }
      };
#endif
      kloop(0, t1, std::true_type{});
      if (sw) {
#pragma unroll
        for (int i = 0; i < TM; ++i) {
          const float f = __builtin_ldexpf(1.0f, eP - (e1s[i] + eB1));
#pragma unroll
          for (int j = 0; j < CT; ++j) acc[i][j] *= f;
        }
      }
      kloop(t1, ntiles, std::false_type{});
    }
    if (kR0XAlias) {
      __syncthreads();
      x_dma();
    }
    {
      const float f = __builtin_ldexpf(1.0f, -eP);
#pragma unroll
      for (int i = 0; i < TM; ++i)
#pragma unroll
        for (int j = 0; j < CT; ++j) acc[i][j] *= f;
    }

    {
      const int tb = Mt * Npad * 4;
      auto mk = [&](const float* p) {
        return __builtin_amdgcn_make_buffer_rsrc((void*)(p + (size_t)t0 * Npad), 0, tb, 0x00020000);
      };
      const __amdgpu_buffer_rsrc_t rH = mk(A.H), rE = mk(kE ? A.E : A.H), rRH = mk(kE ? A.RH : A.H);
      constexpr int EC = R0_EC, LA = kE ? R0_ELA : R0_ELA1;
      float pre[LA + 1][3][EC];
      auto load_part = [&](int c, float (&d)[3][EC]) {
        constexpr int PPT = 16 / EC;
        const int tn = c % CT, tm = (c / CT) / PPT, hf = (c / CT) % PPT;
        const int vo = col0 + 32 * tn < Npad ? ((4 * lh) * Npad + col0 + 32 * tn + lr) * 4 : kOob;
#pragma unroll
        for (int j = 0; j < EC; ++j) {
          const int r = EC * hf + j;
          const int so = (32 * tm + (r & 3) + 8 * (r >> 2)) * Npad * 4;
          if constexpr (R0_ABL == 2) {
            d[0][j] = 0.5f;
            d[1][j] = d[2][j] = 0.25f;
            continue;
          }
          d[0][j] = __builtin_bit_cast(float, __builtin_amdgcn_raw_buffer_load_b32(rH, vo, so, 0));
          if constexpr (kE) {
            d[1][j] = __builtin_bit_cast(float, __builtin_amdgcn_raw_buffer_load_b32(rE, vo, so, 0));
            d[2][j] = __builtin_bit_cast(float, __builtin_amdgcn_raw_buffer_load_b32(rRH, vo, so, 0));
          } else {
            d[1][j] = 0.0f;
            d[2][j] = 0.0f;
          }
        }
      };
      constexpr int NC = (16 / EC) * TM * CT;
#pragma unroll
      for (int c = 0; c < LA && c < NC; ++c) load_part(c, pre[c]);
#pragma unroll
      for (int c = 0; c < NC; ++c) {
        if (c + LA < NC) load_part(c + LA, pre[(c + LA) % (LA + 1)]);
        const float (&op)[3][EC] = pre[c % (LA + 1)];
        const int tn = c % CT, tm = (c / CT) / (16 / EC), hf = (c / CT) % (16 / EC);
#pragma unroll
        for (int j = 0; j < EC; ++j) {
          const int r = EC * hf + j;
          acc[tm][tn][r] = fmaf(op[1][j], op[2][j], acc[tm][tn][r] * one_minus_sq(op[0][j]));
        }
        __builtin_amdgcn_sched_barrier(0);
      }
    }
    float mx = 0.0f;
#pragma unroll
    for (int tn = 0; tn < CT; ++tn)
#pragma unroll
      for (int tm = 0; tm < TM; ++tm)
#pragma unroll
        for (int r = 0; r < 16; ++r) {
          bsum[tn] += acc[tm][tn][r];
          mx = fmaxf(mx, fabsf(acc[tm][tn][r]));
        }
#pragma unroll
    for (int off = 32; off > 0; off >>= 1) mx = fmaxf(mx, __shfl_xor(mx, off, 64));
    if (lane == 0) sMax[w] = mx;
    asm volatile("s_waitcnt vmcnt(0)" ::: "memory");
    __syncthreads();
    float mt = 0.0f;
#pragma unroll
    for (int u = 0; u < kR0NW; ++u) mt = fmaxf(mt, sMax[u]);
    if (R0_ABL != 1 && mt > 0.0f) {
      const int et = f16_scale_exp(mt);
      if (et < Eacc) {
        if (Eacc != (1 << 20)) {
          const float f = __builtin_ldexpf(1.0f, et - Eacc);
#pragma unroll
          for (int i = 0; i < kR0XT; ++i)
#pragma unroll
            for (int j = 0; j < CT; ++j) G[i][j] *= f;
        }
        Eacc = et;
      }
      const float sR = __builtin_ldexpf(1.0f, Eacc);
      const int g4 = lane >> 4, q = (lane >> 2) & 3, pp = lane & 3;
#pragma unroll
      for (int s = 0; s < 2 * TM; ++s) {
        f16x8 bh[CT], bl[CT];
#pragma unroll
        for (int tn = 0; tn < CT; ++tn) {
          float vals[8];
#pragma unroll
          for (int j = 0; j < 8; ++j) vals[j] = acc[s >> 1][tn][8 * (s & 1) + j];
          split8h(vals, sR, bh[tn], bl[tn]);
        }
#pragma unroll
        for (int ot = 0; ot < kR0XT; ++ot) {
          f16x8 xa[2];
#pragma unroll
          for (int pl = 0; pl < 2; ++pl) {
            s8 v;
#pragma unroll
            for (int t = 0; t < 2; ++t) {
              const int row = 16 * s + 8 * t + 4 * (g4 >> 1) + q;
              const int ch = 4 * ot + 2 * (g4 & 1) + (pp >> 1);
              const s4 rr = __builtin_amdgcn_ds_read_tr16_b64_v4i16(
                  (__attribute__((address_space(3))) s4*)(sX + pl * kR0XPL + (xoff(row, ch) >> 1) + 4 * (pp & 1)));
#pragma unroll
              for (int e = 0; e < 4; ++e) v[4 * t + e] = rr[e];
            }
            xa[pl] = __builtin_bit_cast(f16x8, v);
          }
#pragma unroll
          for (int tn = 0; tn < CT; ++tn) G[ot][tn] = mfma3h(xa[0], xa[1], bh[tn], bl[tn], G[ot][tn]);
        }
        __builtin_amdgcn_sched_barrier(0);
      }
    }
    __syncthreads();
  }

  const int lane = tid0 & 63, lr = lane & 31, lh = lane >> 5, col0 = 32 * CT * (tid0 >> 6);
  float* out = A.dst.slab + (size_t)blockIdx.x * A.dst.slab_stride;
  const float fG = Eacc == (1 << 20) ? 0.0f : __builtin_ldexpf(1.0f, -(eX + Eacc));
#pragma unroll
  for (int tn = 0; tn < CT; ++tn) {
    const int j = col0 + 32 * tn + lr;
    if (j < A.N) {
#pragma unroll
      for (int ot = 0; ot < kR0XT; ++ot)
#pragma unroll
        for (int r = 0; r < 16; ++r) {
          const int i = 32 * ot + (r & 3) + 8 * (r >> 2) + 4 * lh;
          if (i < A.obs) out[A.dst.off_w + (int64_t)i * A.N + j] = G[ot][tn][r] * fG;
        }
    }
    const float bt = xadd_f<true>(bsum[tn]);
    if (lh == 0 && j < A.N) out[A.dst.off_b + j] = bt;
  }
}

__device__ __forceinline__ bool rbwd0_sw(const RBwd0Args& A) {
  if (kR0BK != 32 || A.nseg < 2 || !A.A1h || A.low_seg <= 0) return false;
  const int nk = (A.K + kR0BK - 1) / kR0BK;
  if (nk % R0_PF) return false;
  const int q0 = amax_exp(A.am_a0) + amax_exp(A.am_b0), q1 = amax_exp(A.am_a1) + amax_exp(A.am_b1);
  const int pen0 = (!A.am_a0 || !A.am_b0) ? 4 : 0;
  return __builtin_amdgcn_readfirstlane(q1 - q0 >= A.low_seg + pen0 ? 1 : 0) != 0;
}

template <int NSEG>
__global__ void __launch_bounds__(kR0NT, 1) rbwd0_kernel(const RBwd0Args A) {
  __shared__ __attribute__((aligned(16))) unsigned short smem[kR0LDSU];
  __shared__ float sMax[kR0NW];
  if (A.skip && *A.skip) return;
  if constexpr (NSEG > 1) {
    if (rbwd0_sw(A)) {
      rbwd0_body<NSEG, true>(A, smem, sMax);
      return;
    }
  }
  rbwd0_body<NSEG, false>(A, smem, sMax);
}

}

bool rbwd0_eligible(int obs_pad, int x_ldp, int hid_pad, int K) {
  return obs_pad <= 128 && x_ldp <= 128 && hid_pad <= 256 && hid_pad % 32 == 0 && K >= 4 && K % 4 == 0;
}

void launch_rbwd0(const RBwd0Args& a, hipStream_t s) {
  if (a.dst.splits <= 0) return;
  if (!rbwd0_eligible(a.obs, a.x_ldp, a.Npad, a.K) || a.obs > 128 || !a.Xh || !a.Xl || !a.eX || !a.H ||
      (a.nseg > 1 && (!a.A1 || !a.B1)) || (a.E && !a.RH) || a.ldk < (a.K + 15) / 16 * 16 || a.lda < a.K)
    throw std::runtime_error("rbwd0: unsupported shape or missing operand");
  if ((int64_t)a.x_ldp * a.x_mpad * 2 >= (int64_t(1) << 32) || (int64_t)kR0Rows * a.lda * 4 >= (int64_t(1) << 31))
    throw std::runtime_error("rbwd0: operand beyond the buffer-descriptor range");
  if ((int64_t)a.dst.splits * a.dst.rows_per_split < a.rows) throw std::runtime_error("rbwd0: splits do not cover the rows");
  if (a.nseg != 1 && a.nseg != 2) throw std::runtime_error("rbwd0: nseg must be 1 or 2");
  if ((a.nseg == 2) != (a.E != nullptr)) throw std::runtime_error("rbwd0: the E RH term goes with two segments");
  RBwd0Args b = a;
  b.low_seg = g_options.low_seg;
  if (b.nseg == 1) {
    b.A1 = b.A0;
    b.B1 = b.B0;
    b.am_a1 = b.am_a0;
    b.am_b1 = b.am_b0;
  }
  if (a.nseg == 2) hipLaunchKernelGGL(rbwd0_kernel<2>, dim3(a.dst.splits), dim3(kR0NT), 0, s, b);
  else hipLaunchKernelGGL(rbwd0_kernel<1>, dim3(a.dst.splits), dim3(kR0NT), 0, s, b);
}

}
```

trpo_amd/csrc/rfwd.hip:

```cpp
#include "chain_common.h"
#include "rowepi.h"

#include <stdexcept>
#include <type_traits>

namespace trpo {
namespace {

typedef __fp16 rf_h2 __attribute__((ext_vector_type(2)));

#ifndef RF_SGB
#define RF_SGB 1
#endif
#ifndef RF_ILV
#define RF_ILV 1
#endif
#ifndef RF_HOIST
#define RF_HOIST 0
#endif
#ifndef RF_HEAD
#define RF_HEAD 3
#endif
#ifndef RF_CSB
#define RF_CSB 1
#endif
#ifndef RF_ABL
#define RF_ABL 0
#endif

constexpr int kRfUnits = 2048;
constexpr int kRfChunks = 24;
constexpr int kRfLd = 256;
constexpr int kRfTile = 128, kRfWaves = 4;

__device__ __forceinline__ void rf_split8(const float* x, float s, f16x8& hi, f16x8& lo) {
  cu32x4 H, L;
#pragma unroll
  for (int q = 0; q < 4; ++q) {
    const float a = x[2 * q] * s, b = x[2 * q + 1] * s;
    const rf_h2 hp = __builtin_amdgcn_cvt_pkrtz(a, b);
    const rf_h2 lp = __builtin_amdgcn_cvt_pkrtz(a - (float)hp[0], b - (float)hp[1]);
    H[q] = __builtin_bit_cast(unsigned, hp);
    L[q] = __builtin_bit_cast(unsigned, lp);
  }
  hi = __builtin_bit_cast(f16x8, H);
  lo = __builtin_bit_cast(f16x8, L);
}

__device__ __forceinline__ f32x16 rf_mfma3(const f16x8& ah, const f16x8& al, const f16x8& bh, const f16x8& bl,
                                           f32x16 c) {
  c = __builtin_amdgcn_mfma_f32_32x32x16_f16(al, bh, c, 0, 0, 0);
  c = __builtin_amdgcn_mfma_f32_32x32x16_f16(ah, bl, c, 0, 0, 0);
  c = __builtin_amdgcn_mfma_f32_32x32x16_f16(ah, bh, c, 0, 0, 0);
  return c;
}

__global__ void __launch_bounds__(256) rfwd01_img_kernel(const float* __restrict__ theta, const float* __restrict__ v,
                                                         int64_t offV0, int64_t offW1, int obs,
                                                         const unsigned* am_v0, const unsigned* am_w1,
                                                         const unsigned* am_v1, uint16_t* __restrict__ img,
                                                         const int* skip) {
  if (skip && *skip) return;
  const int eV0 = amax_exp(am_v0), eW = amax_exp(am_w1), eV = amax_exp(am_v1);
  const int gid = blockIdx.x * 256 + threadIdx.x;
  const int t = gid / 2560, rem = gid % 2560;
  if (t >= 8) return;
  float x[8];
  cu32x4* dst;
  int plane_units;
  float sc;
  if (rem < 512) {
    const int f = rem >> 4, u = rem & 15, ks = u >> 1, h = u & 1;
#pragma unroll
    for (int q = 0; q < 8; ++q) {
      const int k = 16 * ks + 8 * h + q;
      x[q] = k < obs ? v[offV0 + (int64_t)k * 256 + 32 * t + f] : 0.0f;
    }
    sc = __builtin_ldexpf(1.0f, eV0);
    dst = reinterpret_cast<cu32x4*>(img) + (size_t)(3 * t) * kRfUnits + f * 16 + (u ^ (f & 15));
    plane_units = 512;
  } else {
    const int b = rem - 512, nh = b >> 10, m = (b >> 9) & 1, r = (b >> 2) & 127, u = b & 3, uu = u >> 1, h = u & 1;
    const float* src = m ? v : theta;
#pragma unroll
    for (int q = 0; q < 8; ++q) {
      const int k = 32 * t + 16 * uu + 4 * h + 8 * (q >> 2) + (q & 3);
      x[q] = src[offW1 + (int64_t)k * 256 + 128 * nh + r];
    }
    sc = __builtin_ldexpf(1.0f, m ? eV : eW);
    dst = reinterpret_cast<cu32x4*>(img) + (size_t)(3 * t + 1 + nh) * kRfUnits + m * 1024 + r * 4 +
          (u ^ ((r >> 2) & 3));
    plane_units = 512;
  }
  f16x8 hi, lo;
  rf_split8(x, sc, hi, lo);
  dst[0] = __builtin_bit_cast(cu32x4, hi);
  dst[plane_units] = __builtin_bit_cast(cu32x4, lo);
}

__device__ __forceinline__ void rf_dma16(__amdgpu_buffer_rsrc_t rsrc, unsigned voff, unsigned soff, unsigned lds) {
  unsigned keep;
  asm volatile("s_mov_b32 %0, m0\n\ts_mov_b32 m0, %3\n\ts_nop 0\n\tbuffer_load_dwordx4 %1, %2, 0 offen lds\n\t"
               "s_mov_b32 m0, %0"
               : "=&s"(keep)
               : "v"(voff + soff), "s"(rsrc), "s"(lds));
}

template <int KS0>
__global__ void __launch_bounds__(kRfWaves * 64, 1) rfwd01_kernel(const Rfwd01Args a) {
  static_assert(!RF_ILV || KS0 == 8, "interleaved DMA: one instruction per k-step of phase A");
  __shared__ cu32x4 q0[kRfUnits], q1[kRfUnits], q2[kRfUnits], q3[kRfUnits];
  __shared__ float cvec[2][256];
  __shared__ float red[3][16];
  __shared__ int pex[kRfWaves][32];
  if (a.skip && *a.skip) return;
  const int tid = threadIdx.x, lane = tid & 63, s = lane & 31, h = lane >> 5;
  const int wv = __builtin_amdgcn_readfirstlane(tid >> 6);
  const int eX = __builtin_amdgcn_readfirstlane(*a.eX);
  const int eV0 = __builtin_amdgcn_readfirstlane(amax_exp(a.am_v0));
  const int eW = __builtin_amdgcn_readfirstlane(amax_exp(a.am_w1));
  const int eV = __builtin_amdgcn_readfirstlane(amax_exp(a.am_v1));
  const float uA = __builtin_ldexpf(1.0f, -(eX + eV0));
  const int64_t ntiles = (a.n + kRfTile - 1) / kRfTile;
  const __amdgpu_buffer_rsrc_t rimg =
      __builtin_amdgcn_make_buffer_rsrc((void*)a.img, 0, kRfChunks * kRfUnits * 16, 0x00020000);
  const __amdgpu_buffer_rsrc_t rxh = __builtin_amdgcn_make_buffer_rsrc((void*)a.Xh, 0, 0x7ffffff0, 0x00020000);
  const __amdgpu_buffer_rsrc_t rxl = __builtin_amdgcn_make_buffer_rsrc((void*)a.Xl, 0, 0x7ffffff0, 0x00020000);
  for (int i = tid; i < 256; i += kRfWaves * 64) {
    cvec[0][i] = a.c0[i];
    cvec[1][i] = a.c1[i];
  }
  float nv0 = 0.0f, mc0 = 0.0f;
  if constexpr (RF_CSB) {
    float q = 0.0f;
    for (int k = 0; k < a.obs; ++k) {
      const float x = a.V0[(int64_t)k * 256 + tid];
      q = fmaf(x, x, q);
    }
    float m1 = max32_dpp(sqrtf(q)), m2 = max32_dpp(fabsf(a.c0[tid]));
    m1 = fmaxf(m1, __shfl_xor(m1, 32));
    m2 = fmaxf(m2, __shfl_xor(m2, 32));
    if (lane == 0) {
      red[0][wv] = m1;
      red[1][wv] = m2;
    }
    __syncthreads();
    nv0 = fmaxf(fmaxf(red[0][0], red[0][1]), fmaxf(red[0][2], red[0][3]));
    mc0 = fmaxf(fmaxf(red[1][0], red[1][1]), fmaxf(red[1][2], red[1][3]));
    __syncthreads();
  }
  asm volatile("s_waitcnt vmcnt(0)" ::: "memory");
  auto slot = [&](int k) -> cu32x4* { return k == 0 ? q0 : k == 1 ? q1 : k == 2 ? q2 : q3; };
  auto rows_of = [&](int64_t r0w) { return (int)(a.n - r0w < 32 ? (a.n - r0w > 0 ? a.n - r0w : 0) : 32); };
  auto dma_one = [&](auto A, int c, int sl, int64_t r0w, int i) __attribute__((always_inline)) {
    if constexpr ((RF_ABL & 4) != 0) return;
    const unsigned lds0 = (unsigned)(uintptr_t)slot(sl);
    if (!decltype(A)::value || i < 4) {
      const int base = wv * 64 + i * kRfWaves * 64;
      rf_dma16(rimg, (unsigned)(base + lane) * 16u, (unsigned)c * kRfUnits * 16u, lds0 + (unsigned)base * 16u);
    } else {
      const int t = c / 3, ih = i - 4;
      const __amdgpu_buffer_rsrc_t rh =
          __builtin_amdgcn_make_buffer_rsrc((void*)(a.H1 + r0w * kRfLd), 0, rows_of(r0w) * kRfLd * 4, 0x00020000);
      const int r = 8 * ih + (lane >> 3), cu = (lane & 7) ^ ((r >> 1) & 7);
      rf_dma16(rh, (unsigned)(r * kRfLd + 4 * cu) * 4u, (unsigned)(32 * t) * 4u,
               lds0 + (unsigned)(1024 + wv * 256 + 64 * ih) * 16u);
    }
  };
  auto dma = [&](auto A, int c, int sl, int64_t r0w) __attribute__((always_inline)) {
#pragma unroll
    for (int i = 0; i < 8; ++i) dma_one(A, c, sl, r0w, i);
  };
  using kA = std::true_type;
  using kB = std::false_type;
  auto arrive = [&](bool far, bool first_a0) __attribute__((always_inline)) {
    __builtin_amdgcn_sched_barrier(0);
    if (far) asm volatile("s_waitcnt vmcnt(63)" ::: "memory");
    else if (first_a0 || (RF_ABL & 8) != 0) asm volatile("s_waitcnt vmcnt(16)" ::: "memory");
    else asm volatile("s_waitcnt vmcnt(20)" ::: "memory");
    lds_barrier();
  };
  const unsigned xlane = (unsigned)(s * 32 + 8 * h) * 2u;
  auto xload = [&](int64_t row0, f16x8 (&x)[KS0][2]) __attribute__((always_inline)) {
    if constexpr ((RF_ABL & 16) != 0) {
#pragma unroll
      for (int ks = 0; ks < KS0; ++ks) {
        unsigned u = (unsigned)row0 + ks;
        asm volatile("" : "+v"(u));
        x[ks][0] = x[ks][1] = __builtin_bit_cast(f16x8, cu32x4{u, u, u, u});
      }
      return;
    }
#pragma unroll
    for (int ks = 0; ks < KS0; ++ks) {
      const int so = (int)((((unsigned)(ks >> 1) * (unsigned)a.x_mpad + (unsigned)row0) * 32u + 16u * (ks & 1)) * 2u);
      x[ks][0] = __builtin_bit_cast(f16x8, __builtin_amdgcn_raw_buffer_load_b128(rxh, xlane, so, 0));
      x[ks][1] = __builtin_bit_cast(f16x8, __builtin_amdgcn_raw_buffer_load_b128(rxl, xlane, so, 0));
    }
  };
  const unsigned hlane = (unsigned)(s * kRfLd + 4 * h) * 4u;

  f16x8 xt[KS0][2];
  xload((int64_t)blockIdx.x * kRfTile + wv * 32, xt);
  __builtin_amdgcn_s_waitcnt(0x0f70);
  {
    const int64_t r0f = (int64_t)blockIdx.x * kRfTile + wv * 32;
    dma(kA{}, 0, 0, r0f);
    dma(kB{}, 1, 1, r0f);
    dma(kB{}, 2, 2, r0f);
  }

  float mR = 0.0f, mZ = 0.0f;
  for (int64_t tile = blockIdx.x; tile < ntiles; tile += gridDim.x) {
    const bool first = tile == (int64_t)blockIdx.x;
    const int64_t r0 = tile * kRfTile + wv * 32;
    const int64_t r0n = r0 + (int64_t)gridDim.x * kRfTile;
    const int rows = rows_of(r0);
    const __amdgpu_buffer_rsrc_t rrh =
        __builtin_amdgcn_make_buffer_rsrc((void*)(a.RH1 + r0 * kRfLd), 0, rows * kRfLd * 4, 0x00020000);
    f32x16 acc[8];
#pragma unroll
    for (int i = 0; i < 8; ++i) acc[i] = f32x16{};
    int Ps = 0;
    if constexpr (RF_CSB) {
      float q = 0.0f;
#pragma unroll
      for (int ks = 0; ks < KS0; ++ks) {
        const f16x8 x8 = xt[ks][0];
        q = __builtin_amdgcn_fdot2(__builtin_shufflevector(x8, x8, 0, 1), __builtin_shufflevector(x8, x8, 0, 1), q, false);
        q = __builtin_amdgcn_fdot2(__builtin_shufflevector(x8, x8, 2, 3), __builtin_shufflevector(x8, x8, 2, 3), q, false);
        q = __builtin_amdgcn_fdot2(__builtin_shufflevector(x8, x8, 4, 5), __builtin_shufflevector(x8, x8, 4, 5), q, false);
        q = __builtin_amdgcn_fdot2(__builtin_shufflevector(x8, x8, 6, 7), __builtin_shufflevector(x8, x8, 6, 7), q, false);
      }
      q = xadd_f<true>(q);
      const float bnd = __builtin_ldexpf(sqrtf(q), -eX) * nv0 * 1.01f + mc0;
      Ps = min(bnd > 0.0f ? f16_scale_exp(bnd) + eW : 1000, f16_scale_exp(1.0f) + eV);
    }
    int* px = pex[wv];
#pragma unroll 1
    for (int tq = 0; tq < 2; ++tq) {
#pragma unroll
      for (int tt = 0; tt < 4; ++tt) {
        const int t = 4 * tq + tt;
        const int cA = 3 * t, sA = (3 * tt) % 4;
        const bool far = t == 0 && !first;
        arrive(far, t == 0 && first);
        const int cA3 = cA + 3 < kRfChunks ? cA + 3 : cA + 3 - kRfChunks;
        const int64_t rA3 = cA + 3 < kRfChunks ? r0 : r0n;
        if (!RF_ILV) dma(kA{}, cA3, (sA + 3) % 4, rA3);
        const cu32x4* S = slot(sA);
        float hv[16], cb[16];
        auto ldh = [&]() __attribute__((always_inline)) {
#pragma unroll
          for (int j = 0; j < 4; ++j) {
            const int cu = 2 * j + h;
            const f32x4 v4 = __builtin_bit_cast(f32x4, S[1024 + wv * 256 + s * 8 + (cu ^ ((s >> 1) & 7))]);
#pragma unroll
            for (int i = 0; i < 4; ++i) hv[4 * j + i] = v4[i];
          }
#pragma unroll
          for (int r = 0; r < 16; ++r) cb[r] = cvec[0][32 * t + 8 * (r >> 2) + 4 * h + (r & 3)];
        };
        if (RF_HOIST) ldh();
        f32x16 accA = f32x16{};
        f16x8 fa[2][2];
        auto lda = [&](int ks, f16x8 (&f)[2]) __attribute__((always_inline)) {
          const int au = s * 16 + ((2 * ks + h) ^ (s & 15));
          f[0] = __builtin_bit_cast(f16x8, S[au]);
          f[1] = __builtin_bit_cast(f16x8, S[512 + au]);
        };
        lda(0, fa[0]);
#pragma unroll
        for (int ks = 0; ks < KS0; ++ks) {
          __builtin_amdgcn_sched_barrier(0);
          if (RF_ILV) dma_one(kA{}, cA3, (sA + 3) % 4, rA3, ks);
          if (ks + 1 < KS0) lda(ks + 1, fa[(ks + 1) & 1]);
          if constexpr ((RF_ABL & 32) == 0) accA = rf_mfma3(fa[ks & 1][0], fa[ks & 1][1], xt[ks][0], xt[ks][1], accA);
          if (RF_SGB && ks + 1 < KS0) {
            __builtin_amdgcn_sched_group_barrier(0x100, 2, 0);
            __builtin_amdgcn_sched_group_barrier(0x008, 3, 0);
          }
        }
        __builtin_amdgcn_sched_barrier(0);
        if (!RF_HOIST) ldh();
        float rh[16];
        float mt = 0.0f;
#pragma unroll
        for (int r = 0; r < 16; ++r) {
          if constexpr ((RF_ABL & 64) != 0) {
            rh[r] = accA[r] * uA;
          } else {
            rh[r] = one_minus_sq(hv[r]) * (accA[r] * uA + cb[r]);
            mt = fmaxf(mt, fabsf(rh[r]));
          }
        }
#pragma unroll
        for (int j = 0; j < 4 && (RF_ABL & 8) == 0; ++j)
          __builtin_amdgcn_raw_buffer_store_b128(
              __builtin_bit_cast(cu32x4, f32x4{rh[4 * j], rh[4 * j + 1], rh[4 * j + 2], rh[4 * j + 3]}), rrh, hlane,
              (32 * t + 8 * j) * 4, 0);
        mR = fmaxf(mR, mt);
        if constexpr ((RF_ABL & 64) == 0 && !RF_CSB) mt = xmax_f<true>(mt);
        const int Pt = (RF_ABL & 64) ? 2 : min(mt > 0.0f ? f16_scale_exp(mt) + eW : 1000, f16_scale_exp(1.0f) + eV);
        if constexpr (RF_CSB) {
        } else if (t == 0) {
          Ps = Pt;
        } else if (__builtin_amdgcn_ballot_w64(Pt < Ps - RF_HEAD) != 0) {
          if (h == 0) px[s] = Pt < Ps - RF_HEAD ? Pt - Ps : 0;
          __builtin_amdgcn_wave_barrier();
          __builtin_amdgcn_fence(__ATOMIC_SEQ_CST, "wavefront");
          float f[16];
#pragma unroll
          for (int r = 0; r < 16; ++r) f[r] = __builtin_ldexpf(1.0f, px[8 * (r >> 2) + 4 * h + (r & 3)]);
#pragma unroll
          for (int i = 0; i < 8; ++i)
#pragma unroll
            for (int r = 0; r < 16; ++r) acc[i][r] *= f[r];
          Ps = Pt < Ps - RF_HEAD ? Pt : Ps;
          __builtin_amdgcn_wave_barrier();
        }
        const float sR = __builtin_ldexpf(1.0f, Ps - eW), sH = __builtin_ldexpf(1.0f, Ps - eV);
        f16x8 aR[2][2], aH[2][2];
#pragma unroll
        for (int uu = 0; uu < 2; ++uu) {
          rf_split8(rh + 8 * uu, sR, aR[uu][0], aR[uu][1]);
          rf_split8(hv + 8 * uu, sH, aH[uu][0], aH[uu][1]);
        }
#pragma unroll
        for (int nh = 0; nh < 2; ++nh) {
          const int cB = cA + 1 + nh, sB = (3 * tt + 1 + nh) % 4;
          arrive(far, false);
          const int cB3 = cB + 3 < kRfChunks ? cB + 3 : cB + 3 - kRfChunks;
          const int64_t rB3 = cB + 3 < kRfChunks ? r0 : r0n;
          if (!RF_ILV) dma(kB{}, cB3, (sB + 3) % 4, rB3);
          const cu32x4* B = slot(sB);
          f16x8 fb[2][4];
          auto ldb = [&](int k, f16x8 (&f)[4]) __attribute__((always_inline)) {
            const int col = 32 * (k & 3) + s;
            const int bu = col * 4 + ((2 * (k >> 2) + h) ^ ((col >> 2) & 3));
            f[0] = __builtin_bit_cast(f16x8, B[bu]);
            f[1] = __builtin_bit_cast(f16x8, B[512 + bu]);
            f[2] = __builtin_bit_cast(f16x8, B[1024 + bu]);
            f[3] = __builtin_bit_cast(f16x8, B[1536 + bu]);
          };
          ldb(0, fb[0]);
#pragma unroll
          for (int k = 0; k < 8; ++k) {
            __builtin_amdgcn_sched_barrier(0);
            if (RF_ILV) dma_one(kB{}, cB3, (sB + 3) % 4, rB3, k);
            if (k + 1 < 8 && (RF_ABL & 2) == 0) ldb(k + 1, fb[(k + 1) & 1]);
            const int uu = k >> 2, tn = k & 3;
            const f16x8(&f)[4] = fb[k & 1];
            if ((RF_ABL & 1) == 0) {
              f32x16 c = acc[4 * nh + tn];
              c = rf_mfma3(aR[uu][0], aR[uu][1], f[0], f[1], c);
              c = rf_mfma3(aH[uu][0], aH[uu][1], f[2], f[3], c);
              acc[4 * nh + tn] = c;
            }
            if (RF_SGB && (RF_ABL & 3) == 0 && k + 1 < 8) {
              __builtin_amdgcn_sched_group_barrier(0x100, 4, 0);
              __builtin_amdgcn_sched_group_barrier(0x008, 6, 0);
            }
          }
          __builtin_amdgcn_sched_barrier(0);
        }
      }
    }
    xload(r0n < a.x_mpad ? r0n : 0, xt);
    if (h == 0) px[s] = Ps;
    __builtin_amdgcn_wave_barrier();
    __builtin_amdgcn_fence(__ATOMIC_SEQ_CST, "wavefront");
    float un[16];
#pragma unroll
    for (int r = 0; r < 16; ++r) un[r] = __builtin_ldexpf(1.0f, -px[8 * (r >> 2) + 4 * h + (r & 3)]);
    __builtin_amdgcn_wave_barrier();
    const __amdgpu_buffer_rsrc_t rz =
        __builtin_amdgcn_make_buffer_rsrc((void*)(a.RZ2 + r0 * kRfLd), 0, rows * kRfLd * 4, 0x00020000);
    const unsigned zlane = (unsigned)(4 * h * kRfLd + s) * 4u;
#pragma unroll
    for (int tn = 0; tn < 8; ++tn) {
      const float cn = cvec[1][32 * tn + s];
#pragma unroll
      for (int r = 0; r < 16; ++r) {
        const float o = acc[tn][r] * un[r] + cn;
        mZ = fmaxf(mZ, fabsf(o));
        if constexpr ((RF_ABL & 8) == 0)
          __builtin_amdgcn_raw_buffer_store_b32(__builtin_bit_cast(unsigned, o), rz, zlane,
                                                ((8 * (r >> 2) + (r & 3)) * kRfLd + 32 * tn) * 4, 0);
      }
    }
  }
  asm volatile("s_waitcnt vmcnt(0)" ::: "memory");
  amax_commit3<true>(a.am_rh1, mR, a.am_rz2, mZ, nullptr, 0.0f, red);
}


constexpr int kFwChunks = 16;

__global__ void __launch_bounds__(256) fwd01_img_kernel(const float* __restrict__ th, int64_t offW0, int64_t offW1,
                                                        int obs, const unsigned* am_w0, const unsigned* am_w1,
                                                        uint16_t* __restrict__ img) {
  const int eW0 = amax_exp(am_w0), eW1 = amax_exp(am_w1);
  const int gid = blockIdx.x * 256 + threadIdx.x;
  const int t = gid / 1536, rem = gid % 1536;
  if (t >= 8) return;
  float x[8];
  cu32x4* dst;
  int plane_units;
  float sc;
  if (rem < 512) {
    const int f = rem >> 4, u = rem & 15, ks = u >> 1, h = u & 1;
#pragma unroll
    for (int q = 0; q < 8; ++q) {
      const int k = 16 * ks + 8 * h + q;
      x[q] = k < obs ? th[offW0 + (int64_t)k * 256 + 32 * t + f] : 0.0f;
    }
    sc = __builtin_ldexpf(1.0f, eW0);
    dst = reinterpret_cast<cu32x4*>(img) + (size_t)(2 * t) * kRfUnits + f * 16 + (u ^ (f & 15));
    plane_units = 512;
  } else {
    const int b = rem - 512, r = b >> 2, u = b & 3, uu = u >> 1, h = u & 1;
#pragma unroll
    for (int q = 0; q < 8; ++q) {
      const int k = 32 * t + 16 * uu + 4 * h + 8 * (q >> 2) + (q & 3);
      x[q] = th[offW1 + (int64_t)k * 256 + r];
    }
    sc = __builtin_ldexpf(1.0f, eW1);
    dst = reinterpret_cast<cu32x4*>(img) + (size_t)(2 * t + 1) * kRfUnits + r * 4 + (u ^ ((r >> 2) & 3));
    plane_units = 1024;
  }
  f16x8 hi, lo;
  rf_split8(x, sc, hi, lo);
  dst[0] = __builtin_bit_cast(cu32x4, hi);
  dst[plane_units] = __builtin_bit_cast(cu32x4, lo);
}

template <int KS0, bool PREP>
__global__ void __launch_bounds__(kRfWaves * 64, 1) fwd01_kernel(const Fwd01Args a) {
  __shared__ cu32x4 q0[kRfUnits], q1[kRfUnits], q2[kRfUnits], q3[kRfUnits];
  __shared__ float cvec[2][256];
  const int tid = threadIdx.x, lane = tid & 63, s = lane & 31, h = lane >> 5;
  const int wv = __builtin_amdgcn_readfirstlane(tid >> 6);
  const int eX = __builtin_amdgcn_readfirstlane(*a.eX);
  const int eW0 = __builtin_amdgcn_readfirstlane(amax_exp(a.am_w0));
  const int eW1 = __builtin_amdgcn_readfirstlane(amax_exp(a.am_w1));
  const float uA = __builtin_ldexpf(1.0f, -(eX + eW0));
  const int P = f16_scale_exp(1.0f) + eW1;
  const float sH = __builtin_ldexpf(1.0f, P - eW1), uP = __builtin_ldexpf(1.0f, -P);
  const int64_t ntiles = (a.n + kRfTile - 1) / kRfTile;
  const __amdgpu_buffer_rsrc_t rimg =
      __builtin_amdgcn_make_buffer_rsrc((void*)a.img, 0, kFwChunks * kRfUnits * 16, 0x00020000);
  const __amdgpu_buffer_rsrc_t rxh = __builtin_amdgcn_make_buffer_rsrc((void*)a.Xh, 0, 0x7ffffff0, 0x00020000);
  const __amdgpu_buffer_rsrc_t rxl = __builtin_amdgcn_make_buffer_rsrc((void*)a.Xl, 0, 0x7ffffff0, 0x00020000);
  for (int i = tid; i < 256; i += kRfWaves * 64) {
    cvec[0][i] = a.b0[i];
    cvec[1][i] = a.b1[i];
  }
  asm volatile("s_waitcnt vmcnt(0)" ::: "memory");
  auto slot = [&](int k) -> cu32x4* { return k == 0 ? q0 : k == 1 ? q1 : k == 2 ? q2 : q3; };
  auto rows_of = [&](int64_t r0w) { return (int)(a.n - r0w < 32 ? (a.n - r0w > 0 ? a.n - r0w : 0) : 32); };
  auto dma_one = [&](int c, int sl, int i) __attribute__((always_inline)) {
    const unsigned lds0 = (unsigned)(uintptr_t)slot(sl);
    const int base = wv * 64 + i * kRfWaves * 64;
    rf_dma16(rimg, (unsigned)(base + lane) * 16u, (unsigned)c * kRfUnits * 16u, lds0 + (unsigned)base * 16u);
  };
  constexpr int S = PREP ? 4 : 0;
  auto arrive = [&](int cnt) __attribute__((always_inline)) {
    __builtin_amdgcn_sched_barrier(0);
    if (cnt >= 63) asm volatile("s_waitcnt vmcnt(63)" ::: "memory");
    else if (PREP && cnt == 20) asm volatile("s_waitcnt vmcnt(20)" ::: "memory");
    else if (PREP && cnt == 16) asm volatile("s_waitcnt vmcnt(16)" ::: "memory");
    else asm volatile("s_waitcnt vmcnt(12)" ::: "memory");
    lds_barrier();
  };
  const unsigned xlane = (unsigned)(s * 32 + 8 * h) * 2u;
// ... 55 lines not shown
        }
        __builtin_amdgcn_sched_barrier(0);
        float hv[16];
#pragma unroll
        for (int r = 0; r < 16; ++r)
          hv[r] = tanh_fast(accA[r] * uA + cvec[0][32 * t + 8 * (r >> 2) + 4 * h + (r & 3)]);
        if constexpr (PREP) {
          const __amdgpu_buffer_rsrc_t rh1 =
              __builtin_amdgcn_make_buffer_rsrc((void*)(a.H1 + r0 * kRfLd), 0, rows * kRfLd * 4, 0x00020000);
#pragma unroll
          for (int j = 0; j < 4; ++j)
            __builtin_amdgcn_raw_buffer_store_b128(
                __builtin_bit_cast(cu32x4, f32x4{hv[4 * j], hv[4 * j + 1], hv[4 * j + 2], hv[4 * j + 3]}), rh1,
                hlane, (32 * t + 8 * j) * 4, 0);
        }
        f16x8 aH[2][2];
#pragma unroll
        for (int uu = 0; uu < 2; ++uu) rf_split8(hv + 8 * uu, sH, aH[uu][0], aH[uu][1]);
        arrive(!first && t == 0 ? 63 : (first && t == 0 ? 12 + S : 12 + 2 * S));
        const int cB3 = cB + 3 < kFwChunks ? cB + 3 : cB + 3 - kFwChunks;
        const cu32x4* B = slot(sB);
        f16x8 fb[2][2];
        auto ldb = [&](int k, f16x8 (&f)[2]) __attribute__((always_inline)) {
          const int col = 128 * (k >> 3) + 32 * (k & 3) + s;
          const int bu = col * 4 + ((2 * ((k >> 2) & 1) + h) ^ ((col >> 2) & 3));
          f[0] = __builtin_bit_cast(f16x8, B[bu]);
          f[1] = __builtin_bit_cast(f16x8, B[1024 + bu]);
        };
        ldb(0, fb[0]);
#pragma unroll
        for (int k = 0; k < 16; ++k) {
          __builtin_amdgcn_sched_barrier(0);
          if (k < 4) dma_one(cB3, (sB + 3) % 4, k);
          if (k + 1 < 16) ldb(k + 1, fb[(k + 1) & 1]);
          const int uu = (k >> 2) & 1, tn = k & 3, nh = k >> 3;
          acc[4 * nh + tn] = rf_mfma3(aH[uu][0], aH[uu][1], fb[k & 1][0], fb[k & 1][1], acc[4 * nh + tn]);
          if (RF_SGB && k + 1 < 16) {
            __builtin_amdgcn_sched_group_barrier(0x100, 2, 0);
            __builtin_amdgcn_sched_group_barrier(0x008, 3, 0);
          }
        }
        __builtin_amdgcn_sched_barrier(0);
      }
    }
    xload(r0n < a.x_mpad ? r0n : 0, xt);
    const __amdgpu_buffer_rsrc_t rz =
        __builtin_amdgcn_make_buffer_rsrc((void*)(a.H2 + r0 * kRfLd), 0, rows * kRfLd * 4, 0x00020000);
    const unsigned zlane = (unsigned)(4 * h * kRfLd + s) * 4u;
#pragma unroll
    for (int tn = 0; tn < 8; ++tn) {
      const float bn = cvec[1][32 * tn + s];
#pragma unroll
      for (int r = 0; r < 16; ++r)
        __builtin_amdgcn_raw_buffer_store_b32(__builtin_bit_cast(unsigned, tanh_fast(acc[tn][r] * uP + bn)), rz,
                                              zlane, ((8 * (r >> 2) + (r & 3)) * kRfLd + 32 * tn) * 4, 0);
    }
  }
  asm volatile("s_waitcnt vmcnt(0)" ::: "memory");
}

}

bool rfwd01_eligible(int L, const int* w, const int* wp) {
  return L == 3 && w[0] >= 1 && w[0] <= 128 && w[1] == 256 && w[2] == 256 && wp[1] == 256 && wp[2] == 256;
}

size_t rfwd01_img_bytes() { return (size_t)kRfChunks * kRfUnits * 16; }

void launch_rfwd01_img(const float* theta, const float* v, int64_t offV0, int64_t offW1, int obs,
                       const unsigned* am_v0, const unsigned* am_w1, const unsigned* am_v1, uint16_t* img,
                       const int* skip, hipStream_t s) {
  hipLaunchKernelGGL(rfwd01_img_kernel, dim3(8 * 2560 / 256), dim3(256), 0, s, theta, v, offV0, offW1, obs, am_v0,
                     am_w1, am_v1, img, skip);
}

void launch_rfwd01(const Rfwd01Args& a, int num_cus, hipStream_t s) {
  if (a.n <= 0) return;
  if (a.obs < 1 || a.obs > 128 || a.ldh != 256 || a.ldz != 256)
    throw std::runtime_error("rfwd01: unsupported shape");
  if (!rfwd01_rows_ok(a.x_mpad) || a.x_mpad < (a.n + kRfTile - 1) / kRfTile * kRfTile)
    throw std::runtime_error("rfwd01: X plane geometry");
  const int64_t ntiles = (a.n + kRfTile - 1) / kRfTile;
  const int grid = (int)std::min<int64_t>(ntiles, (int64_t)num_cus);
  hipLaunchKernelGGL(rfwd01_kernel<8>, dim3(grid), dim3(kRfWaves * 64), 0, s, a);
}

bool fwd01_eligible(int L, const int* w, const int* wp) { return rfwd01_eligible(L, w, wp); }

size_t fwd01_img_bytes() { return (size_t)kFwChunks * kRfUnits * 16; }

void launch_fwd01_img(const float* th, int64_t offW0, int64_t offW1, int obs, const unsigned* am_w0,
                      const unsigned* am_w1, uint16_t* img, hipStream_t s) {
  hipLaunchKernelGGL(fwd01_img_kernel, dim3(8 * 1536 / 256), dim3(256), 0, s, th, offW0, offW1, obs, am_w0, am_w1,
                     img);
}

void launch_fwd01(const Fwd01Args& a, int num_cus, hipStream_t s) {
  if (a.n <= 0) return;
  if (a.obs < 1 || a.obs > 128) throw std::runtime_error("fwd01: unsupported shape");
  if (!rfwd01_rows_ok(a.x_mpad) || a.x_mpad < (a.n + kRfTile - 1) / kRfTile * kRfTile)
    throw std::runtime_error("fwd01: X plane geometry");
  const int64_t ntiles = (a.n + kRfTile - 1) / kRfTile;
  const int grid = (int)std::min<int64_t>(ntiles, (int64_t)num_cus);
  if (a.H1) hipLaunchKernelGGL((fwd01_kernel<8, true>), dim3(grid), dim3(kRfWaves * 64), 0, s, a);
  else hipLaunchKernelGGL((fwd01_kernel<8, false>), dim3(grid), dim3(kRfWaves * 64), 0, s, a);
}

}
```

trpo_amd/csrc/standalone.cpp:

```cpp
#include "../../include/trpo_engine.h"
#include "abi_util.h"
#include "kernels.h"

#include <hip/hip_runtime.h>

#include <cstring>
#include <string>

using namespace trpo;
using namespace trpo_abi;

extern "C" {

void trpo_default_params(trpo_update_params* p) {
  if (!p) return;
  p->cg_iters = 10;
  p->residual_tol = 1e-10f;
  p->cg_damping = 0.1f;
  p->max_kl = 0.01;
  p->compute_advantages = 0;
  p->gamma = 0.95;
}

void trpo_default_rollout_params(trpo_rollout_params* p) {
// ... 30 lines not shown
    st.fetch();
    HIPCHECK(hipDeviceSynchronize());
  });
}

int trpo_cartpole_step(const double* state, const int64_t* action, int64_t n, double* state_out, double* reward,
                       uint8_t* done, int mem) {
  return guarded([&] {
    REQUIRE(state && action && state_out && n >= 0, "bad argument");
    if (n == 0) return;
    Staging st(mem, nullptr);
    const double* ds = st.in(state, (size_t)n * 4);
    const int64_t* da = st.in(action, (size_t)n);
    double* dso = st.out(state_out, (size_t)n * 4);
    double* dr = st.out(reward, (size_t)n);
    launch_cartpole_step(ds, da, n, dso, dr, st.out(done, (size_t)n), nullptr);
    check_launch();
    st.fetch();
    HIPCHECK(hipDeviceSynchronize());
  });
}

int trpo_discount(const double* x, const uint8_t* starts, int64_t n, double gamma, double* out, int mem) {
  return guarded([&] {
    REQUIRE(x && out, "NULL argument");
    REQUIRE(n >= 0, "n < 0");
    if (n == 0) return;
    Staging st(mem, nullptr);
    const double* dx = st.in(x, (size_t)n);
    const uint8_t* ds = st.in(starts, (size_t)n);
    if (!ds) {
      uint8_t* z = st.tmp<uint8_t>((size_t)n);
      HIPCHECK(hipMemset(z, 0, (size_t)n));
      ds = z;
    }
    launch_discount(dx, ds, n, gamma, st.out(out, (size_t)n), st.tmp<uint8_t>(discount_workspace_bytes(n)), nullptr);
    check_launch();
    HIPCHECK(hipDeviceSynchronize());
    st.fetch();
  });
}

int trpo_gae(const double* rewards, const double* values, const uint8_t* starts, const double* tail_values,
             int64_t n, double gamma, double lambda, double* adv_out, double* returns_out, int mem) {
  return guarded([&] {
    REQUIRE(n >= 0, "n < 0");
    REQUIRE(lambda >= 0.0 && lambda <= 1.0, "lambda must be in [0, 1]");
    if (n == 0) return;
    REQUIRE(rewards, "rewards is NULL");
    Staging st(mem, nullptr);
    const double* dr = st.in(rewards, (size_t)n);
    const double* dv = st.in(values, (size_t)n);
    const uint8_t* ds = st.in(starts, (size_t)n);
    const double* dt = st.in(tail_values, (size_t)n);
    double* da = st.out(adv_out, (size_t)n);
    double* dret = st.out(returns_out, (size_t)n);
    launch_gae(dr, dv, ds, dt, n, gamma, lambda, da, dret, st.tmp<uint8_t>(gae_workspace_bytes(n)), nullptr);
    check_launch();
    HIPCHECK(hipDeviceSynchronize());
    st.fetch();
  });
}

static int* option_slot(const std::string& k) {
  if (k == "split_mfma") return &g_options.split_mfma;
  if (k == "split_wg") return &g_options.split_wg;
  if (k == "chain") return &g_options.chain;
  if (k == "split_f16") return &g_options.split_f16;
  if (k == "split_min_k") return &g_options.split_min_k;
  if (k == "graphs") return &g_options.graphs;
  if (k == "tail") return &g_options.tail;
  if (k == "fused") return &g_options.fused;
  if (k == "low_seg") return &g_options.low_seg;
  if (k == "planes") return &g_options.planes;
  if (k == "rbwd0") return &g_options.rbwd0;
  if (k == "hbwd2") return &g_options.hbwd2;
  if (k == "head_fwd") return &g_options.head_fwd;
  if (k == "splits") return &g_options.splits;
  if (k == "pg_splits") return &g_options.pg_splits;
  if (k == "ls_fused") return &g_options.ls_fused;
  if (k == "cg_fuse_reduce") return &g_options.cg_fuse_reduce;
  if (k == "rfwd01") return &g_options.rfwd01;
  if (k == "fwd01") return &g_options.fwd01;
  if (k == "cg_p_img") return &g_options.cg_p_img;
  throw ArgError("unknown option " + k);
}

int trpo_set_option(const char* name, int value) {
  return guarded([&] {
    REQUIRE(name, "NULL argument");
    *option_slot(name) = value;
  });
}

int trpo_get_option(const char* name, int* value) {
  return guarded([&] {
    REQUIRE(name && value, "NULL argument");
    *value = *option_slot(name);
  });
}

}
```

Baseline: 2.433 updates/s.

## Store FVP R-forward hidden activation RH1 as scaled f16 hi/lo pair planes

The fused rfwd01 kernel now writes the layer-1 R-op activation as two f16 planes (hi and residual lo) in a row-paired 256-column layout with a shared power-of-two scale, instead of fp32. The rbwd0 backward kernel and the split-f16 wgrad kernel read these planes directly, so RH1 traffic is halved and the later kernels skip re-splitting fp32 into f16. When the one-segment path applies, the lo plane is not read at all. This adds a new layout, pairing of odd row counts, a bound-derived exponent and extra validation checks, and accuracy depends on that bound being correct.

```diff
diff --git a/include/trpo_engine.h b/include/trpo_engine.h
--- a/include/trpo_engine.h
+++ b/include/trpo_engine.h
@@ -115,6 +115,7 @@
              double* returns_out, int mem);
 
 int trpo_set_option(const char* name, int value);
+int trpo_plane_rows_ok(int64_t x_mpad, int* rfwd01_ok, int* pair_planes_ok);
 int trpo_get_option(const char* name, int* value);
 
 int trpo_profile_enable(trpo_engine* e, int enable);
diff --git a/trpo_amd/_lib.py b/trpo_amd/_lib.py
--- a/trpo_amd/_lib.py
+++ b/trpo_amd/_lib.py
@@ -97,6 +97,7 @@
     "trpo_gae": (c_int, [c_void_p, c_void_p, c_void_p, c_void_p, c_int64, c_double, c_double, c_void_p, c_void_p,
                          c_int]),
     "trpo_set_option": (c_int, [c_char_p, c_int]),
+    "trpo_plane_rows_ok": (c_int, [c_int64, POINTER(c_int), POINTER(c_int)]),
     "trpo_get_option": (c_int, [c_char_p, POINTER(c_int)]),
     "trpo_profile_enable": (c_int, [c_void_p, c_int]),
     "trpo_profile_query": (c_int, [c_void_p, c_char_p, c_int]),
diff --git a/trpo_amd/csrc/engine.cpp b/trpo_amd/csrc/engine.cpp
--- a/trpo_amd/csrc/engine.cpp
+++ b/trpo_amd/csrc/engine.cpp
@@ -187,6 +187,14 @@
   bool use_rbwd0() const {
     return g_options.rbwd0 != 0 && f16 && x_planes_on() && rbwd0_geom() && rowgemm_uses_split(wp[1], RowEpi::kRBwd);
   }
+  bool use_rh1_planes() const {
+    return g_options.rh1_planes != 0 && use_rfwd01() && use_rbwd0() && g_options.split_wg != 0 &&
+           wp[1] == kPairLd && pair_planes_rows_ok(x_mpad);
+  }
+  PairPlane rh1_planes() const {
+    const unsigned* hi = reinterpret_cast<const unsigned*>(RH[1]);
+    return PairPlane{hi, hi + pair_plane_dwords(n), pl_e + 2};
+  }
   RBwd0Args rbwd0_args(const int* skip) const {
     RBwd0Args a{};
     a.rows = (int)n;
@@ -371,7 +379,7 @@
     E.assign(L, nullptr);
     for (int l = 1; l < L; ++l) {
       H[l] = dalloc<float>((size_t)cap * wp[l]);
-      RH[l] = dalloc<float>((size_t)cap * wp[l]);
+      RH[l] = dalloc<float>((size_t)(cap + (cap & 1)) * wp[l]);
     }
     for (int l = 0; l < L; ++l) {
       D[l] = dalloc<float>((size_t)cap * wp[l + 1]);
@@ -1093,13 +1101,15 @@
     launch_wgrad(a, stream);
     check_launch();
   }
-  void fvp_wgrads(int l0, int l1, const int* skip) {
+  void fvp_wgrads(int l0, int l1, const int* skip, bool rh1p = false) {
     for (int l = l0; l < l1; ++l) {
-      if (l == 0)
+      if (l == 0) {
         wgrad_layer(0, 1, WSeg{X, RD[0], wp[0], wp[1], am_x(), am_rd(0)}, WSeg{}, 0, skip, "fvp_wgrad");
-      else
-        wgrad_layer(l, 2, WSeg{RH[l], D[l], wp[l], wp[l + 1], am_rh(l), am_d(l)},
-                    WSeg{H[l], RD[l], wp[l], wp[l + 1], nullptr, am_rd(l)}, 1, skip, "fvp_wgrad");
+      } else {
+        WSeg s0{RH[l], D[l], wp[l], wp[l + 1], am_rh(l), am_d(l)};
+        if (l == 1 && rh1p) s0.Ap = rh1_planes();
+        wgrad_layer(l, 2, s0, WSeg{H[l], RD[l], wp[l], wp[l + 1], nullptr, am_rd(l)}, 1, skip, "fvp_wgrad");
+      }
     }
   }
 
@@ -1179,6 +1189,7 @@
     const bool tail = use_tail();
     const int Lf = tail ? L - 1 : L;
     int l_first = 0;
+    const bool rh1p = use_rh1_planes();
     if (use_rfwd01()) {
       {
         Scope sp(this, "fvp_rfwd_img");
@@ -1206,6 +1217,7 @@
       ra.am_v1 = am_v(1);
       ra.am_rh1 = am_rh(1);
       ra.am_rz2 = am_rh(2);
+      if (rh1p) ra.e_rh1 = pl_e + 2;
       ra.skip = skip;
       Scope sp(this, "fvp_rfwd01");
       launch_rfwd01(ra, num_cus, stream);
@@ -1300,6 +1312,7 @@
         a.am_a1 = am_d(1);
         a.E = E[0];
         a.RH = RH[1];
+        if (rh1p) a.RHp = rh1_planes();
         Scope sp(this, "fvp_rbwdwg_l1");
         launch_rbwd0(a, stream);
         check_launch();
@@ -1321,7 +1334,7 @@
       launch_rowgemm(a, stream);
       check_launch();
     }
-    fvp_wgrads(r0f ? 1 : 0, Lf, skip);
+    fvp_wgrads(r0f ? 1 : 0, Lf, skip, rh1p);
     reduce_grad(out, skip);
   }
 
diff --git a/trpo_amd/csrc/gemm.hip b/trpo_amd/csrc/gemm.hip
--- a/trpo_amd/csrc/gemm.hip
+++ b/trpo_amd/csrc/gemm.hip
@@ -20,7 +20,8 @@
                      env_int("TRPO_HEAD_FWD", 1), env_int("TRPO_SPLITS", 0),
                      env_int("TRPO_PG_SPLITS", 0), env_int("TRPO_LS_FUSED", 1),
                      env_int("TRPO_CG_FUSE_REDUCE", 1), env_int("TRPO_CG_P_IMG", 1),
-                     env_int("TRPO_RFWD01", 1), env_int("TRPO_FWD01", 1)};
+                     env_int("TRPO_RFWD01", 1), env_int("TRPO_FWD01", 1),
+                     env_int("TRPO_RH1_PLANES", 1)};
 
 namespace {
 
@@ -427,9 +428,10 @@
 }
 
 
-template <int WM, int WN, int TM, int TN, int OCC, int PF, int NP>
+template <int WM, int WN, int TM, int TN, int OCC, int PF, int NP, bool PA = false>
 __global__ void __launch_bounds__(WM* WN * 64, OCC)
 wgrad3_kernel(const WGradArgs args) {
+  static_assert(!PA || NP == 2, "plane operands are f16");
   constexpr int BK = 16;
   constexpr int BM = WM * TM * 32, BN = WN * TN * 32, NT = WM * WN * 64;
   constexpr int APL = BM * BK, BPL = BN * BK;
@@ -463,6 +465,7 @@
       one0 = -d >= args.low_seg + pen1;
       one1 = d >= args.low_seg + pen0;
     }
+    if constexpr (PA) eA[0] = __builtin_amdgcn_readfirstlane(*args.seg[0].Ap.e);
   }
 
   f32x16 acc[TM][TN];
@@ -509,14 +512,36 @@
     const int kt = t - sg * nk;
     st.cs = do_colsum && sg == args.colsum_seg;
     st.sg = sg;
-    const __amdgpu_buffer_rsrc_t ra = desc(sg ? args.seg[1].A : args.seg[0].A, args.seg[0].lda);
     const __amdgpu_buffer_rsrc_t rb = desc(sg ? args.seg[1].B : args.seg[0].B, args.seg[0].ldb);
     const int sa = kt * BK * lda4, sb = kt * BK * ldb4;
-    __builtin_amdgcn_sched_barrier(0);
-#pragma unroll
-    for (int i = 0; i < AP; ++i)
-#pragma unroll
-      for (int q = 0; q < 8; ++q) st.va[i][q] = ldbuf(ra, vA[i], sa + q * lda4);
+    if constexpr (PA) {
+      const bool p0 = sg == 0;
+      const size_t pair0 = (size_t)(r0 >> 1) * kPairLd;
+      const float* const fa = args.seg[1].A + (size_t)r0 * args.seg[0].lda;
+      const void* const b03 = p0 ? (const void*)(args.seg[0].Ap.hi + pair0) : (const void*)fa;
+      const void* const b47 = p0 ? (const void*)(args.seg[0].Ap.lo + pair0) : (const void*)fa;
+      const int bytes = p0 ? (r1 - r0 + 1) / 2 * kPairLd * 4 : (r1 - r0) * lda4;
+      const __amdgpu_buffer_rsrc_t r03 = __builtin_amdgcn_make_buffer_rsrc((void*)b03, 0, bytes, 0x00020000);
+      const __amdgpu_buffer_rsrc_t r47 = __builtin_amdgcn_make_buffer_rsrc((void*)b47, 0, bytes, 0x00020000);
+      const int s0 = p0 ? sa / 2 : sa, sq = p0 ? kPairLd * 4 : lda4, s4 = p0 ? s0 : sa + 4 * lda4;
+      __builtin_amdgcn_sched_barrier(0);
+#pragma unroll
+      for (int i = 0; i < AP; ++i) {
+        const int v03 = p0 ? vA[i] - ((vA[i] >> 1) & (4 * kPairLd * 4)) : vA[i];
+        const int v47 = (p0 && one0) ? kOob : v03;
+#pragma unroll
+        for (int q = 0; q < 4; ++q) st.va[i][q] = ldbuf(r03, v03, s0 + q * sq);
+#pragma unroll
+        for (int q = 0; q < 4; ++q) st.va[i][4 + q] = ldbuf(r47, v47, s4 + q * sq);
+      }
+    } else {
+      const __amdgpu_buffer_rsrc_t ra = desc(sg ? args.seg[1].A : args.seg[0].A, args.seg[0].lda);
+      __builtin_amdgcn_sched_barrier(0);
+#pragma unroll
+      for (int i = 0; i < AP; ++i)
+#pragma unroll
+        for (int q = 0; q < 8; ++q) st.va[i][q] = ldbuf(ra, vA[i], sa + q * lda4);
+    }
 #pragma unroll
     for (int i = 0; i < BP; ++i)
 #pragma unroll
@@ -558,7 +583,18 @@
 #pragma unroll
     for (int i = 0; i < AP; ++i) {
       const int f = tid + i * NT;
-      if (AI % NT == 0 || f < AI) put(As, APL, f % BM, f / BM, st.va[i], eA[st.sg]);
+      if (AI % NT != 0 && f >= AI) continue;
+      if (PA && st.sg == 0) {
+        typedef unsigned u32x4s __attribute__((ext_vector_type(4)));
+        unsigned short* dst = As + swz16(f % BM, f / BM);
+        *reinterpret_cast<u32x4s*>(dst) = u32x4s{__float_as_uint(st.va[i][0]), __float_as_uint(st.va[i][1]),
+                                                 __float_as_uint(st.va[i][2]), __float_as_uint(st.va[i][3])};
+        if (!one0)
+          *reinterpret_cast<u32x4s*>(dst + APL) = u32x4s{__float_as_uint(st.va[i][4]), __float_as_uint(st.va[i][5]),
+                                                         __float_as_uint(st.va[i][6]), __float_as_uint(st.va[i][7])};
+      } else {
+        put(As, APL, f % BM, f / BM, st.va[i], eA[st.sg]);
+      }
     }
 #pragma unroll
     for (int i = 0; i < BP; ++i) {
@@ -990,9 +1026,18 @@
   if ((int64_t)a.dst.rows_per_split * (a.seg[0].lda > a.seg[0].ldb ? a.seg[0].lda : a.seg[0].ldb) * 4 >= (int64_t(1) << 30))
     throw std::runtime_error("split-bf16 wgrad: a split's rows exceed the 1 GiB buffer-descriptor range");
   dim3 grid((a.Ma + BM - 1) / BM, (a.Nb + BN - 1) / BN, a.dst.splits);
+  if (a.nseg > 1 && a.seg[1].Ap.hi) throw std::runtime_error("split-f16 wgrad: only segment 0 takes planes");
+  if (a.seg[0].Ap.hi && (!a.f16 || a.nseg != 2 || !a.seg[0].Ap.lo || !a.seg[0].Ap.e || a.seg[0].lda != kPairLd ||
+                         a.Mpad > kPairLd))
+    throw std::runtime_error("split-f16 wgrad: plane operand needs the f16 split, two segments, both planes and 256 columns");
   WGradArgs b = a;
   b.low_seg = g_options.low_seg;
-  if (a.f16)
+  if (a.f16 && a.seg[0].Ap.hi) {
+    if constexpr (BM == kPairLd)
+      hipLaunchKernelGGL((wgrad3_kernel<WM, WN, TM, TN, OCC, 2, 2, true>), grid, dim3(WM * WN * 64), 0, s, b);
+    else
+      throw std::runtime_error("split-f16 wgrad: plane operand on a tile narrower than its 256 columns");
+  } else if (a.f16)
     hipLaunchKernelGGL((wgrad3_kernel<WM, WN, TM, TN, OCC, PF, 2>), grid, dim3(WM * WN * 64), 0, s, b);
   else
     hipLaunchKernelGGL((wgrad3_kernel<WM, WN, TM, TN, OCC, PF, 3>), grid, dim3(WM * WN * 64), 0, s, a);
@@ -1042,6 +1087,8 @@
 void launch_wgrad(const WGradArgs& a, hipStream_t s) {
   if (a.dst.splits <= 0) return;
   const int Mp = a.Ma, Np = a.Nb;
+  if ((a.seg[0].Ap.hi || (a.nseg > 1 && a.seg[1].Ap.hi)) && (Np <= 128 || g_options.split_wg == 0))
+    throw std::runtime_error("wgrad: plane operand outside the split kernel");
   if (Np <= 32) {
     if (Mp <= 64) launch_wg_cfg<2, 1, 1, 1>(a, s);
     else if (Mp <= 128) launch_wg_cfg<4, 1, 1, 1>(a, s);
diff --git a/trpo_amd/csrc/kernels.h b/trpo_amd/csrc/kernels.h
--- a/trpo_amd/csrc/kernels.h
+++ b/trpo_amd/csrc/kernels.h
@@ -25,6 +25,7 @@
   int cg_p_img;
   int rfwd01;
   int fwd01;
+  int rh1_planes;
 };
 
 constexpr int kAmaxSub = 256, kAmaxStride = 32, kAmaxSlot = kAmaxSub * kAmaxStride;
@@ -129,12 +130,21 @@
   int64_t off_w = 0, off_b = 0;
 };
 
+struct PairPlane {
+  const unsigned* hi = nullptr;
+  const unsigned* lo = nullptr;
+  const int* e = nullptr;
+};
+constexpr int kPairLd = 256;
+constexpr int64_t pair_plane_dwords(int64_t rows) { return (rows + 1) / 2 * kPairLd; }
+
 struct WSeg {
   const float* A;
   const float* B;
   int lda, ldb;
   const unsigned* amaxA = nullptr;
   const unsigned* amaxB = nullptr;
+  PairPlane Ap{};
 };
 
 struct WGradArgs {
@@ -417,6 +427,7 @@
   const float* H;
   const float* E;
   const float* RH;
+  PairPlane RHp{};
   const uint16_t* Xh;
   const uint16_t* Xl;
   int x_mpad, x_ldp;
@@ -475,6 +486,7 @@
   const float *H1, *c0, *c1;
   const float* V0;
   float *RH1, *RZ2;
+  int* e_rh1 = nullptr;
   const uint16_t* img;
   const unsigned *am_v0, *am_w1, *am_v1;
   unsigned *am_rh1, *am_rz2;
@@ -493,6 +505,7 @@
 };
 constexpr bool rfwd01_rows_ok(int64_t x_mpad) { return 4 * x_mpad * 64 < (int64_t(1) << 31); }
 static_assert(rfwd01_rows_ok((1 << 23) - 256) && !rfwd01_rows_ok(1 << 23), "rfwd01 / fwd01 row limit");
+constexpr bool pair_planes_rows_ok(int64_t x_mpad) { return rfwd01_rows_ok(x_mpad); }
 bool fwd01_eligible(int L, const int* w, const int* wp);
 size_t fwd01_img_bytes();
 void launch_fwd01_img(const float* th, int64_t offW0, int64_t offW1, int obs, const unsigned* am_w0,
diff --git a/trpo_amd/csrc/rbwd0.hip b/trpo_amd/csrc/rbwd0.hip
--- a/trpo_amd/csrc/rbwd0.hip
+++ b/trpo_amd/csrc/rbwd0.hip
@@ -97,7 +97,7 @@
   return __builtin_amdgcn_mfma_f32_32x32x16_f16(ah, bh, c, 0, 0, 0);
 }
 
-template <int NSEG, bool SW>
+template <int NSEG, bool SW, int RP>
 __device__ __forceinline__ void rbwd0_body(const RBwd0Args& A, unsigned short* smem, float* sMax) {
   constexpr bool kE = NSEG == 2;
   constexpr int TM = kR0TM, CT = kR0CT;
@@ -122,7 +122,6 @@
 
   const int nk = (K + kR0BK - 1) / kR0BK;
   const int ntiles = NSEG * nk;
-  (void)one1;
   constexpr int sw = SW ? 1 : 0;
   const int eA1p = (sw && !A.eA1t) ? __builtin_amdgcn_readfirstlane(*A.eA1p) : 0;
   const int bbytes = (int)(2 * A.plane * 2);
@@ -354,13 +353,22 @@
       auto mk = [&](const float* p) {
         return __builtin_amdgcn_make_buffer_rsrc((void*)(p + (size_t)t0 * Npad), 0, tb, 0x00020000);
       };
-      const __amdgpu_buffer_rsrc_t rH = mk(A.H), rE = mk(kE ? A.E : A.H), rRH = mk(kE ? A.RH : A.H);
+      const __amdgpu_buffer_rsrc_t rH = mk(A.H), rE = mk(kE ? A.E : A.H), rRH = mk(kE && !RP ? A.RH : A.H);
+      auto mkp = [&](const unsigned* p) {
+        return __builtin_amdgcn_make_buffer_rsrc((void*)(p + (size_t)(t0 >> 1) * kPairLd), 0,
+                                                 (Mt + 1) / 2 * kPairLd * 4, 0x00020000);
+      };
+      const __amdgpu_buffer_rsrc_t rPh = RP ? mkp(A.RHp.hi) : rH, rPl = RP == 2 ? mkp(A.RHp.lo) : rH;
+      const bool lo2 = RP == 2 && !one1;
+      const float uR = RP ? __builtin_ldexpf(1.0f, -__builtin_amdgcn_readfirstlane(*A.RHp.e)) : 1.0f;
       constexpr int EC = R0_EC, LA = kE ? R0_ELA : R0_ELA1;
+      static_assert(!RP || EC % 2 == 0, "a plane dword holds two accumulator registers");
       float pre[LA + 1][3][EC];
       auto load_part = [&](int c, float (&d)[3][EC]) {
         constexpr int PPT = 16 / EC;
         const int tn = c % CT, tm = (c / CT) / PPT, hf = (c / CT) % PPT;
         const int vo = col0 + 32 * tn < Npad ? ((4 * lh) * Npad + col0 + 32 * tn + lr) * 4 : kOob;
+        const int vp = vo - ((vo >> 1) & (2 * kPairLd * 4));
 #pragma unroll
         for (int j = 0; j < EC; ++j) {
           const int r = EC * hf + j;
@@ -373,13 +381,28 @@
           d[0][j] = __builtin_bit_cast(float, __builtin_amdgcn_raw_buffer_load_b32(rH, vo, so, 0));
           if constexpr (kE) {
             d[1][j] = __builtin_bit_cast(float, __builtin_amdgcn_raw_buffer_load_b32(rE, vo, so, 0));
-            d[2][j] = __builtin_bit_cast(float, __builtin_amdgcn_raw_buffer_load_b32(rRH, vo, so, 0));
+            if constexpr (RP == 0) {
+              d[2][j] = __builtin_bit_cast(float, __builtin_amdgcn_raw_buffer_load_b32(rRH, vo, so, 0));
+            } else if ((j & 1) == 0) {
+              const int sp = (16 * tm + ((r & 3) >> 1) + 4 * (r >> 2)) * kPairLd * 4;
+              d[2][j >> 1] = __builtin_bit_cast(float, __builtin_amdgcn_raw_buffer_load_b32(rPh, vp, sp, 0));
+              if constexpr (RP == 2)
+                d[2][EC / 2 + (j >> 1)] =
+                    __builtin_bit_cast(float, __builtin_amdgcn_raw_buffer_load_b32(rPl, lo2 ? vp : kOob, sp, 0));
+            }
           } else {
             d[1][j] = 0.0f;
             d[2][j] = 0.0f;
           }
         }
       };
+      auto plane_rh = [&](const float (&d)[3][EC], int j) {
+        typedef _Float16 h2 __attribute__((ext_vector_type(2)));
+        auto half = [&](float w) { return (float)__builtin_bit_cast(h2, w)[j & 1]; };
+        float v = half(d[2][j >> 1]);
+        if constexpr (RP == 2) v += half(d[2][EC / 2 + (j >> 1)]);
+        return v * uR;
+      };
       constexpr int NC = (16 / EC) * TM * CT;
 #pragma unroll
       for (int c = 0; c < LA && c < NC; ++c) load_part(c, pre[c]);
@@ -391,7 +414,10 @@
 #pragma unroll
         for (int j = 0; j < EC; ++j) {
           const int r = EC * hf + j;
-          acc[tm][tn][r] = fmaf(op[1][j], op[2][j], acc[tm][tn][r] * one_minus_sq(op[0][j]));
+          float rhv;
+          if constexpr (kE && RP != 0) rhv = plane_rh(op, j);
+          else rhv = op[2][j];
+          acc[tm][tn][r] = fmaf(op[1][j], rhv, acc[tm][tn][r] * one_minus_sq(op[0][j]));
         }
         __builtin_amdgcn_sched_barrier(0);
       }
@@ -484,27 +510,37 @@
   }
 }
 
-__device__ __forceinline__ bool rbwd0_sw(const RBwd0Args& A) {
+__device__ __forceinline__ bool rbwd0_one1(const RBwd0Args& A) {
+  if (A.nseg < 2 || A.low_seg <= 0) return false;
+  const int q0 = amax_exp(A.am_a0) + amax_exp(A.am_b0), q1 = amax_exp(A.am_a1) + amax_exp(A.am_b1);
+  const int pen0 = (!A.am_a0 || !A.am_b0) ? 4 : 0;
+  return __builtin_amdgcn_readfirstlane(q1 - q0 >= A.low_seg + pen0 ? 1 : 0) != 0;
+}
+__device__ __forceinline__ bool rbwd0_sw(const RBwd0Args& A, bool one1) {
   if (kR0BK != 32 || A.nseg < 2 || !A.A1h || A.low_seg <= 0) return false;
   const int nk = (A.K + kR0BK - 1) / kR0BK;
   if (nk % R0_PF) return false;
-  const int q0 = amax_exp(A.am_a0) + amax_exp(A.am_b0), q1 = amax_exp(A.am_a1) + amax_exp(A.am_b1);
-  const int pen0 = (!A.am_a0 || !A.am_b0) ? 4 : 0;
-  return __builtin_amdgcn_readfirstlane(q1 - q0 >= A.low_seg + pen0 ? 1 : 0) != 0;
-}
-
-template <int NSEG>
+  return one1;
+}
+
+template <int NSEG, bool PL = false>
 __global__ void __launch_bounds__(kR0NT, 1) rbwd0_kernel(const RBwd0Args A) {
   __shared__ __attribute__((aligned(16))) unsigned short smem[kR0LDSU];
   __shared__ float sMax[kR0NW];
   if (A.skip && *A.skip) return;
   if constexpr (NSEG > 1) {
-    if (rbwd0_sw(A)) {
-      rbwd0_body<NSEG, true>(A, smem, sMax);
+    const bool one1 = rbwd0_one1(A), sw = rbwd0_sw(A, one1);
+    if constexpr (PL) {
+      if (sw) rbwd0_body<NSEG, true, 1>(A, smem, sMax);
+      else rbwd0_body<NSEG, false, 2>(A, smem, sMax);
       return;
     }
+    if (sw) {
+      rbwd0_body<NSEG, true, 0>(A, smem, sMax);
+      return;
+    }
   }
-  rbwd0_body<NSEG, false>(A, smem, sMax);
+  rbwd0_body<NSEG, false, 0>(A, smem, sMax);
 }
 
 }
@@ -523,6 +559,8 @@
   if ((int64_t)a.dst.splits * a.dst.rows_per_split < a.rows) throw std::runtime_error("rbwd0: splits do not cover the rows");
   if (a.nseg != 1 && a.nseg != 2) throw std::runtime_error("rbwd0: nseg must be 1 or 2");
   if ((a.nseg == 2) != (a.E != nullptr)) throw std::runtime_error("rbwd0: the E RH term goes with two segments");
+  if (a.RHp.hi && (a.nseg != 2 || !a.RHp.lo || !a.RHp.e || a.Npad != kPairLd || a.dst.rows_per_split % 2))
+    throw std::runtime_error("rbwd0: RH_1 planes need two segments, both planes and 256 columns");
   RBwd0Args b = a;
   b.low_seg = g_options.low_seg;
   if (b.nseg == 1) {
@@ -531,7 +569,8 @@
     b.am_a1 = b.am_a0;
     b.am_b1 = b.am_b0;
   }
-  if (a.nseg == 2) hipLaunchKernelGGL(rbwd0_kernel<2>, dim3(a.dst.splits), dim3(kR0NT), 0, s, b);
+  if (a.nseg == 2 && a.RHp.hi) hipLaunchKernelGGL((rbwd0_kernel<2, true>), dim3(a.dst.splits), dim3(kR0NT), 0, s, b);
+  else if (a.nseg == 2) hipLaunchKernelGGL(rbwd0_kernel<2>, dim3(a.dst.splits), dim3(kR0NT), 0, s, b);
   else hipLaunchKernelGGL(rbwd0_kernel<1>, dim3(a.dst.splits), dim3(kR0NT), 0, s, b);
 }
 
diff --git a/trpo_amd/csrc/rfwd.hip b/trpo_amd/csrc/rfwd.hip
--- a/trpo_amd/csrc/rfwd.hip
+++ b/trpo_amd/csrc/rfwd.hip
@@ -106,7 +106,7 @@
                : "v"(voff + soff), "s"(rsrc), "s"(lds));
 }
 
-template <int KS0>
+template <int KS0, bool PL>
 __global__ void __launch_bounds__(kRfWaves * 64, 1) rfwd01_kernel(const Rfwd01Args a) {
   static_assert(!RF_ILV || KS0 == 8, "interleaved DMA: one instruction per k-step of phase A");
   __shared__ cu32x4 q0[kRfUnits], q1[kRfUnits], q2[kRfUnits], q3[kRfUnits];
@@ -149,6 +149,16 @@
     mc0 = fmaxf(fmaxf(red[1][0], red[1][1]), fmaxf(red[1][2], red[1][3]));
     __syncthreads();
   }
+  int eR = 0;
+  if constexpr (PL) {
+    static_assert(RF_CSB, "the planes' exponent comes from the bound");
+    const float bnd = sqrtf((float)a.obs) * __builtin_ldexpf(1.0f, 12 - eX) * nv0 * 1.01f + mc0;
+    eR = __builtin_amdgcn_readfirstlane(f16_scale_exp(bnd));
+    if (blockIdx.x == 0 && tid == 0) *a.e_rh1 = eR;
+  }
+  const float scR = __builtin_ldexpf(1.0f, eR);
+  const bool odd = (s & 1) != 0;
+  const unsigned plane_lo = (unsigned)pair_plane_dwords(a.n);
   asm volatile("s_waitcnt vmcnt(0)" ::: "memory");
   auto slot = [&](int k) -> cu32x4* { return k == 0 ? q0 : k == 1 ? q1 : k == 2 ? q2 : q3; };
   auto rows_of = [&](int64_t r0w) { return (int)(a.n - r0w < 32 ? (a.n - r0w > 0 ? a.n - r0w : 0) : 32); };
@@ -198,7 +208,8 @@
       x[ks][1] = __builtin_bit_cast(f16x8, __builtin_amdgcn_raw_buffer_load_b128(rxl, xlane, so, 0));
     }
   };
-  const unsigned hlane = (unsigned)(s * kRfLd + 4 * h) * 4u;
+  const unsigned hlane = PL ? (unsigned)((s >> 1) * kPairLd + 16 * (s & 1) + 4 * h) * 4u
+                            : (unsigned)(s * kRfLd + 4 * h) * 4u;
 
   f16x8 xt[KS0][2];
   xload((int64_t)blockIdx.x * kRfTile + wv * 32, xt);
@@ -217,7 +228,7 @@
     const int64_t r0n = r0 + (int64_t)gridDim.x * kRfTile;
     const int rows = rows_of(r0);
     const __amdgpu_buffer_rsrc_t rrh =
-        __builtin_amdgcn_make_buffer_rsrc((void*)(a.RH1 + r0 * kRfLd), 0, rows * kRfLd * 4, 0x00020000);
+        __builtin_amdgcn_make_buffer_rsrc((void*)(a.RH1 + r0 * kRfLd), 0, PL ? 0 : rows * kRfLd * 4, 0x00020000);
     f32x16 acc[8];
 #pragma unroll
     for (int i = 0; i < 8; ++i) acc[i] = f32x16{};
@@ -294,11 +305,39 @@
             mt = fmaxf(mt, fabsf(rh[r]));
           }
         }
-#pragma unroll
-        for (int j = 0; j < 4 && (RF_ABL & 8) == 0; ++j)
-          __builtin_amdgcn_raw_buffer_store_b128(
-              __builtin_bit_cast(cu32x4, f32x4{rh[4 * j], rh[4 * j + 1], rh[4 * j + 2], rh[4 * j + 3]}), rrh, hlane,
-              (32 * t + 8 * j) * 4, 0);
+        if constexpr (PL) {
+          float* const ph = a.RH1 + (r0 >> 1) * kPairLd;
+          int pbytes = (rows + 1) / 2 * kPairLd * 4;
+          asm volatile("" : "+s"(pbytes));
+          const __amdgpu_buffer_rsrc_t rph = __builtin_amdgcn_make_buffer_rsrc((void*)ph, 0, pbytes, 0x00020000);
+          const __amdgpu_buffer_rsrc_t rpl =
+              __builtin_amdgcn_make_buffer_rsrc((void*)(ph + plane_lo), 0, pbytes, 0x00020000);
+#pragma unroll
+          for (int j = 0; j < 2; ++j) {
+            cu32x4 Hq, Lq;
+#pragma unroll
+            for (int q = 0; q < 4; ++q) {
+              const int i = 4 * j + q;
+              const float nl = dpp_f<kDppX1>(rh[i]), nh = dpp_f<kDppX1>(rh[8 + i]);
+              const float ev = (odd ? nh : rh[i]) * scR, od = (odd ? rh[8 + i] : nl) * scR;
+              const rf_h2 hp = __builtin_amdgcn_cvt_pkrtz(ev, od);
+              const rf_h2 lp = __builtin_amdgcn_cvt_pkrtz(ev - (float)hp[0], od - (float)hp[1]);
+              Hq[q] = __builtin_bit_cast(unsigned, hp);
+              Lq[q] = __builtin_bit_cast(unsigned, lp);
+            }
+            if constexpr ((RF_ABL & 8) == 0) {
+              __builtin_amdgcn_raw_buffer_store_b128(Hq, rph, hlane, (32 * t + 8 * j) * 4, 0);
+              __builtin_amdgcn_raw_buffer_store_b128(Lq, rpl, hlane, (32 * t + 8 * j) * 4, 0);
+            }
+            __builtin_amdgcn_sched_barrier(0);
+          }
+        } else {
+#pragma unroll
+          for (int j = 0; j < 4 && (RF_ABL & 8) == 0; ++j)
+            __builtin_amdgcn_raw_buffer_store_b128(
+                __builtin_bit_cast(cu32x4, f32x4{rh[4 * j], rh[4 * j + 1], rh[4 * j + 2], rh[4 * j + 3]}), rrh, hlane,
+                (32 * t + 8 * j) * 4, 0);
+        }
         mR = fmaxf(mR, mt);
         if constexpr ((RF_ABL & 64) == 0 && !RF_CSB) mt = xmax_f<true>(mt);
         const int Pt = (RF_ABL & 64) ? 2 : min(mt > 0.0f ? f16_scale_exp(mt) + eW : 1000, f16_scale_exp(1.0f) + eV);
@@ -391,6 +430,16 @@
     }
   }
   asm volatile("s_waitcnt vmcnt(0)" ::: "memory");
+  if constexpr (PL) {
+    if ((a.n & 1) != 0 && (int64_t)blockIdx.x == (ntiles - 1) % (int64_t)gridDim.x) {
+      __syncthreads();
+      int col = threadIdx.x;
+      asm volatile("" : "+v"(col));
+      unsigned short* const p = reinterpret_cast<unsigned short*>(a.RH1 + (a.n >> 1) * kPairLd + col) + 1;
+      p[0] = 0;
+      p[2 * pair_plane_dwords(a.n)] = 0;
+    }
+  }
   amax_commit3<true>(a.am_rh1, mR, a.am_rz2, mZ, nullptr, 0.0f, red);
 }
 
@@ -612,7 +661,12 @@
     throw std::runtime_error("rfwd01: X plane geometry");
   const int64_t ntiles = (a.n + kRfTile - 1) / kRfTile;
   const int grid = (int)std::min<int64_t>(ntiles, (int64_t)num_cus);
-  hipLaunchKernelGGL(rfwd01_kernel<8>, dim3(grid), dim3(kRfWaves * 64), 0, s, a);
+  if (a.e_rh1) {
+    if (!pair_planes_rows_ok(a.x_mpad)) throw std::runtime_error("rfwd01: RH1 plane geometry");
+    hipLaunchKernelGGL((rfwd01_kernel<8, true>), dim3(grid), dim3(kRfWaves * 64), 0, s, a);
+  } else {
+    hipLaunchKernelGGL((rfwd01_kernel<8, false>), dim3(grid), dim3(kRfWaves * 64), 0, s, a);
+  }
 }
 
 bool fwd01_eligible(int L, const int* w, const int* wp) { return rfwd01_eligible(L, w, wp); }
diff --git a/trpo_amd/csrc/standalone.cpp b/trpo_amd/csrc/standalone.cpp
--- a/trpo_amd/csrc/standalone.cpp
+++ b/trpo_amd/csrc/standalone.cpp
@@ -136,8 +136,17 @@
   if (k == "cg_fuse_reduce") return &g_options.cg_fuse_reduce;
   if (k == "rfwd01") return &g_options.rfwd01;
   if (k == "fwd01") return &g_options.fwd01;
+  if (k == "rh1_planes") return &g_options.rh1_planes;
   if (k == "cg_p_img") return &g_options.cg_p_img;
   throw ArgError("unknown option " + k);
+}
+
+int trpo_plane_rows_ok(int64_t x_mpad, int* rfwd01_ok, int* pair_planes_ok) {
+  return guarded([&] {
+    REQUIRE(rfwd01_ok && pair_planes_ok, "NULL argument");
+    *rfwd01_ok = rfwd01_rows_ok(x_mpad) ? 1 : 0;
+    *pair_planes_ok = pair_planes_rows_ok(x_mpad) ? 1 : 0;
+  });
 }
 
 int trpo_set_option(const char* name, int value) {
```

Result: faster. 2.469 updates/s (median of 6 runs) (+1.5%).
